# andewx/dieselfluid

Measured on AMD Instinct MI355X. Metric: M particle-steps/sec, 16M-particle WCSPH dam-break; % HBM roofline, higher is better.
Workload: dtype f32; 1 GPU; WCSPH dam-break, 16003008 particles (n3=252), h=2dx, uniform-grid neighbours, density + pressure/viscosity force + integrate + walls, math=fast; particles=16003008, parallelism=single GPU

## Files before the change

bindings/go/dslsph/dslsph.go:

```go
package dslsph

import "C"

import (
	"errors"
	"fmt"
	"unsafe"
)

var bufferIDs = map[string]C.int{
	"positions":  C.DSL_BUF_POSITIONS,
	"velocities": C.DSL_BUF_VELOCITIES,
	"forces":     C.DSL_BUF_FORCES,
	"densities":  C.DSL_BUF_DENSITIES,
	"pressures":  C.DSL_BUF_PRESSURES,
	"temps":      C.DSL_BUF_PCI_POSITIONS,
}

var auxBuffers = map[string]bool{"sizes": true, "floats": true, "sampler": true, "vecs": true}

type Engine struct {
	h      *C.dsl_handle
	Params C.dsl_params
}
// ... 323 lines not shown
	default:
		rc = C.DSL_ERR_INVALID
	}
	if rc == 0 {
		rc = C.dsl_sync(h)
	}
	if rc == 0 {
		x <- 103
	} else {
		x <- 102
	}
}

func (cp *ComputeGPU) PassIntBuffer(cpu_buffer []int, name string) error {
	if !auxBuffers[name] {
		return cp.isregistered(name)
	}
	p := &cp.eng.Params
	if name == "sizes" && len(cpu_buffer) >= 2 && (C.int32_t(cpu_buffer[0]) != p.n_particles || C.int32_t(cpu_buffer[1]) != p.n_boundary) {
		return errors.New("sizes block {N, Nboundary, ..} does not match the engine's parameters")
	}
	cp.log += "Passed Integer Buffer " + name + "\n"
	return nil
}
func (cp *ComputeGPU) ReadIntBuffer(cpu_buffer []int, name string) error {
	p := &cp.eng.Params
	switch name {
	case "sizes":
		v := [4]int{int(p.n_particles), int(p.n_boundary), int(p.lsh_buckets), int(p.lsh_bucket_size)}
		copy(cpu_buffer, v[:])
		return nil
	case "sampler":
		t := make([]int32, len(cpu_buffer))
		if len(t) == 0 {
			return nil
		}
		if err := cp.eng.ck(C.dsl_lsh_download_table(cp.eng.h, (*C.int32_t)(unsafe.Pointer(&t[0])), C.size_t(len(t)))); err != nil {
			return err
		}
		for k := range t {
			cpu_buffer[k] = int(t[k])
		}
		return nil
	}
	return fmt.Errorf("buffer [%s] holds no integers", name)
}

func (cp *ComputeGPU) RegisterGLBuffer(gl_buffer_id uint32, size int, name string) error {
	if name != "positions" {
		return errors.New("only the positions buffer has a render hand-off")
	}
	cp.registered[name] = size
	cp.log += fmt.Sprintf("RegisterGLBuffer() - buffer %s (GL id %d): read the device arrays through DevicePointers()\n", name, gl_buffer_id)
	return nil
}

func (cp *ComputeGPU) RegisterKernel(name string) bool {
	ok := name == "compute_density" || name == "predict_correct"
	if ok {
		cp.kernels[name] = true
	}
	return ok
}
func (cp *ComputeGPU) Set(d Descriptor)       { *cp.desc = d }
func (cp *ComputeGPU) Get() Descriptor        { return *cp.desc }
func (cp *ComputeGPU) HasDeviceContext() bool { return cp.eng != nil && cp.eng.h != nil }
func (cp *ComputeGPU) ValidState() bool       { return cp.HasDeviceContext() }
func (cp *ComputeGPU) Log() string            { return cp.log }


func Version() string { return C.GoString(C.dsl_version()) }

func (e *Engine) GetParams() (C.dsl_params, error) {
	var p C.dsl_params
	err := e.ck(C.dsl_get_params(e.h, &p))
	return p, err
}
const (
	OptSkin            = int(C.DSL_OPT_SKIN)
	OptSkinSteps       = int(C.DSL_OPT_SKIN_STEPS)
	OptSkinRebuilds    = int(C.DSL_OPT_SKIN_REBUILDS)
	OptSkinSuspensions = int(C.DSL_OPT_SKIN_SUSPENSIONS)
	OptSkinPredict     = int(C.DSL_OPT_SKIN_PREDICT)
	OptDeviceBytes     = int(C.DSL_OPT_DEVICE_BYTES)
	OptGridOversub     = int(C.DSL_OPT_GRID_OVERSUB)
	OptColliderTriangles = int(C.DSL_OPT_COLLIDER_TRIANGLES)
	OptCollideHits       = int(C.DSL_OPT_COLLIDE_HITS)
	OptCollideCull       = int(C.DSL_OPT_COLLIDE_CULL)
	OptCollideIndex        = int(C.DSL_OPT_COLLIDE_INDEX)
	OptCollideIndexEdge    = int(C.DSL_OPT_COLLIDE_INDEX_EDGE)
	OptCollideIndexCells   = int(C.DSL_OPT_COLLIDE_INDEX_CELLS)
	OptCollideIndexEntries = int(C.DSL_OPT_COLLIDE_INDEX_ENTRIES)
	OptCollideVisits       = int(C.DSL_OPT_COLLIDE_VISITS)
	OptCollideFullWaves    = int(C.DSL_OPT_COLLIDE_FULL_WAVES)
	OptCollideSlab = int(C.DSL_OPT_COLLIDE_SLAB)
)

func (e *Engine) SetOption(option int, value float64) error {
	return e.ck(C.dsl_set_option(e.h, C.int(option), C.double(value)))
}
func (e *Engine) GetOption(option int) (float64, error) {
	var v C.double
	err := e.ck(C.dsl_get_option(e.h, C.int(option), &v))
	return float64(v), err
}

func (e *Engine) ResetForces() error { return e.ck(C.dsl_reset_forces(e.h)) }
func (e *Engine) ForcePass() error   { return e.ck(C.dsl_force_pass(e.h)) }

func (e *Engine) SetStream(hipStream unsafe.Pointer) error { return e.ck(C.dsl_set_stream(e.h, hipStream)) }
func (e *Engine) UseOwnStream() error                      { return e.ck(C.dsl_use_own_stream(e.h)) }

func (e *Engine) Count() (live, owned int, err error) {
	var a, b C.int
	err = e.ck(C.dsl_get_count(e.h, &a, &b))
	return int(a), int(b), err
}

func (e *Engine) TimingEnable(mode int) error { return e.ck(C.dsl_timing_enable(e.h, C.int(mode))) }
func (e *Engine) TimingReset() error          { return e.ck(C.dsl_timing_reset(e.h)) }
func (e *Engine) Timing(kernelID int) (avgMs float64, launches int64, err error) {
	var ms C.double
	var n C.int64_t
	err = e.ck(C.dsl_timing_get(e.h, C.int(kernelID), &ms, &n))
	return float64(ms), int64(n), err
}

func (e *Engine) DownloadSorted(buffer C.int, out []float32) error {
	return e.ck(C.dsl_download_sorted(e.h, buffer, (*C.float)(unsafe.Pointer(&out[0])), C.size_t(len(out))))
}
func (e *Engine) DownloadIDs(out []int32) error {
	return e.ck(C.dsl_download_ids(e.h, (*C.int32_t)(unsafe.Pointer(&out[0])), C.size_t(len(out))))
}
func (e *Engine) DownloadCellStart(out []int32) error {
	return e.ck(C.dsl_download_cell_start(e.h, (*C.int32_t)(unsafe.Pointer(&out[0])), C.size_t(len(out))))
}

func SlabMessageFloats(capFull, capX int) int {
	return int(C.dsl_slab_message_floats(C.int(capFull), C.int(capX)))
}
func (e *Engine) SlabMessageFloats(capFull, capX int) int {
	return int(C.dsl_slab_message_floats_for(e.h, C.int(capFull), C.int(capX)))
}
func (e *Engine) SlabRecordFloats() int { return int(C.dsl_slab_record_floats(e.h)) }
func (e *Engine) SlabSplit(width, margin float32) error {
	return e.ck(C.dsl_slab_split(e.h, C.float(width), C.float(margin)))
}
func (e *Engine) ForcePassSplit(phase int) error { return e.ck(C.dsl_force_pass_split(e.h, C.int(phase))) }
func (e *Engine) SlabPack(widthFull, width float32, devLo, devHi unsafe.Pointer, capFull, capX int) error {
	return e.ck(C.dsl_slab_pack(e.h, C.float(widthFull), C.float(width), (*C.float)(devLo), (*C.float)(devHi), C.int(capFull), C.int(capX)))
}
func (e *Engine) SlabPackBand(widthFull float32, devLo, devHi unsafe.Pointer, capFull, capX int, stream unsafe.Pointer) error {
	return e.ck(C.dsl_slab_pack_band(e.h, C.float(widthFull), (*C.float)(devLo), (*C.float)(devHi), C.int(capFull), C.int(capX), stream))
}
func (e *Engine) SlabAppend(devMsg unsafe.Pointer, capFull, capX int) error {
	return e.ck(C.dsl_slab_append(e.h, (*C.float)(devMsg), C.int(capFull), C.int(capX)))
}
func (e *Engine) SlabAppend2(devMsgA, devMsgB unsafe.Pointer, capFull, capX int) error {
	return e.ck(C.dsl_slab_append2(e.h, (*C.float)(devMsgA), (*C.float)(devMsgB), C.int(capFull), C.int(capX)))
}

func (e *Engine) SlabStatus(resetHighWater bool) (st [4]int32, err error) {
	r := C.int(0)
	if resetHighWater {
		r = 1
	}
// ... 130 lines not shown
```

dieselfluid_amd/csrc/dslsph.hip:

```cpp
#include "../../include/dslsph.h"

#include <hip/hip_runtime.h>

#include <algorithm>
#include <climits>
#include <cmath>
#include <cstdio>
#include <cstdlib>
#include <cstring>
#include <new>
#include <string>
#include <type_traits>
#include <utility>
#include <vector>

#include "kernels_lsh.hpp"
#include "kernels_tiled.hpp"
#include "kernels_skin.hpp"
#include "engine.hpp"

using namespace dsl;

namespace {
std::string g_create_error;
// ... 538 lines not shown
    hipLaunchKernelGGL(k_update, dim3(grid_for(launch_n(h))), dim3(kBlock), 0, h->stream, c, bnd_of(h), p, v, f, uni, h->dstats,
                       xs);
  });
  if (rc) return rc;
  h->col_stage = 1;
  h->forces_uniform = true;
  h->press_zero = true;
  h->grid_valid = false;
  h->masks_valid = false;
  return DSL_OK;
}

int host_count(dsl_handle* h, int* out) {
  if (!h->c.n_ptr) {
    *out = h->n;
    return DSL_OK;
  }
  HIP_TRY(h, hipMemcpyAsync(out, h->dn, sizeof(int), hipMemcpyDeviceToHost, h->stream));
  HIP_TRY(h, hipStreamSynchronize(h->stream));
  h->n = *out;
  return DSL_OK;
}

struct BufArrays {
  int comps;
  float* a[3];
};
BufArrays buf_arrays(dsl_handle* h, int buffer) {
  auto three = [](Soa3 s) { return BufArrays{3, {s.x, s.y, s.z}}; };
  switch (buffer) {
    case DSL_BUF_POSITIONS: return three(mpos(h, h->cur_pv));
    case DSL_BUF_VELOCITIES: return three(mvel(h, h->cur_pv));
    case DSL_BUF_FORCES: return three(mfrc(h));
    case DSL_BUF_PCI_POSITIONS: return three(mpcip(h));
    case DSL_BUF_PCI_VELOCITIES: return three(mpciv(h));
    case DSL_BUF_DENSITIES: return BufArrays{1, {h->rho, nullptr, nullptr}};
    case DSL_BUF_PRESSURES: return BufArrays{1, {h->press, nullptr, nullptr}};
    default: return BufArrays{0, {nullptr, nullptr, nullptr}};
  }
}

void free_all(dsl_handle* h) {
  for (int w = 0; w < 2; ++w) {
    for (int k = 0; k < 6; ++k) {
      (void)hipFree(h->pv[w][k]);
      (void)hipFree(h->pci[w][k]);
    }
    for (int k = 0; k < 3; ++k) (void)hipFree(h->frc[w][k]);
    if (w == 0)
      for (int k = 0; k < 3; ++k) {
        (void)hipFree(h->gterm[k]);
        (void)hipFree(h->xsph[k]);
      }
    (void)hipFree(h->ids[w]);
  }
  (void)hipFree(h->rho);
  (void)hipFree(h->pterm);
  (void)hipFree(h->press);
  (void)hipFree(h->scratch1);
  (void)hipFree(h->rank);
  (void)hipFree(h->sort_keys);
  (void)hipFree(h->cell_keys_alloc);
  (void)hipFree(h->sort_work);
  (void)hipFree(h->unordered);
  (void)hipFree(h->cell_count);
  (void)hipFree(h->cell_start);
  (void)hipFree(h->block_sums);
  (void)hipFree(h->qcount);
  (void)hipFree(h->qstart);
  (void)hipFree(h->qsums);
  (void)hipFree(h->qrec);
  (void)hipFree(h->qtiles);
  (void)hipFree(h->n_qtiles);
  (void)hipFree(h->qtile_desc);
  (void)hipFree(h->qrows);
  (void)hipFree(h->qslot);
  (void)hipFree(h->pci_drift);
  if (h->pci_drift_host) (void)hipHostFree(h->pci_drift_host);
  if (h->ev_drift) (void)hipEventDestroy(h->ev_drift);
  (void)hipFree(h->skin_state);
  (void)hipFree(h->walk_ctr);
  (void)hipFree(h->lists);
  for (int k = 0; k < 6; ++k) (void)hipFree(h->pvz[k]);
  for (int k = 0; k < 3; ++k) (void)hipFree(h->pvr[k]);
  (void)hipFree(h->stage);
  (void)hipFree(h->dstats);
  (void)hipFree(h->dcounter);
  (void)hipFree(h->dn);
  (void)hipFree(h->pack_counts);
  (void)hipFree(h->tiles);
  (void)hipFree(h->tile_desc_of);
  (void)hipFree(h->tile_desc);
  (void)hipFree(h->n_tiles);
  (void)hipFree(h->hashv);
  (void)hipFree(h->bucket_of);
  (void)hipFree(h->lsh_table);
  (void)hipFree(h->lsh_len);
  (void)hipFree(h->lsh_samples);
  (void)hipFree(h->nmask);
  (void)hipFree(h->col_rec);
  (void)hipFree(h->col_box);
  (void)hipFree(h->col_chunk);
  (void)hipFree(h->col_hits);
  (void)hipFree(h->col_query);
  col_index_free(h);
  for (hipEvent_t e : h->pool) (void)hipEventDestroy(e);
  for (auto& v : h->pending)
    for (auto& pr : v) {
      (void)hipEventDestroy(pr.first);
      (void)hipEventDestroy(pr.second);
    }
  if (h->ev_band) (void)hipEventDestroy(h->ev_band);
  if (h->own_stream) (void)hipStreamDestroy(h->own_stream);
}

int alloc_pci(dsl_handle* h) {
  for (int k = 0; k < 3; ++k)
    if (!h->gterm[k])
      if (int rc = dev_alloc(h, &h->gterm[k], (size_t)h->cap)) return rc;
  for (int k = 0; k < 3; ++k)
    if (!h->xsph[k])
      if (int rc = dev_alloc(h, &h->xsph[k], (size_t)h->cap)) return rc;
  for (int w = 0; w < 2; ++w)
    for (int k = 0; k < 6; ++k)
      if (!h->pci[w][k])
        if (int rc = dev_alloc(h, &h->pci[w][k], (size_t)h->cap)) return rc;
  if (!h->pci_drift)
    if (int rc = dev_alloc(h, &h->pci_drift, (size_t)512)) return rc;
  if (!h->pci_drift_host) HIP_TRY(h, hipHostMalloc((void**)&h->pci_drift_host, 512 * sizeof(unsigned int), hipHostMallocDefault));
  if (!h->ev_drift) HIP_TRY(h, hipEventCreateWithFlags(&h->ev_drift, hipEventDisableTiming));
  return DSL_OK;
}

bool pci_tiled(const dsl_handle* h);
int alloc_query_bins(dsl_handle* h) {
  int rc = DSL_OK;
  if (!h->qcount && (rc = dev_alloc(h, &h->qcount, (size_t)h->ncell_pad))) return rc;
  if (!h->qstart && (rc = dev_alloc(h, &h->qstart, (size_t)h->ncell_pad))) return rc;
  if (!h->qsums && (rc = dev_alloc(h, &h->qsums, (size_t)h->nscan))) return rc;
  if (!h->qrec && (rc = dev_alloc(h, &h->qrec, (size_t)h->cap))) return rc;
  if (pci_tiled(h)) {
    if (!h->qtiles && (rc = dev_alloc(h, &h->qtiles, (size_t)h->tg.ntiles))) return rc;
    if (!h->n_qtiles && (rc = dev_alloc(h, &h->n_qtiles, (size_t)8))) return rc;
    if (!h->qtile_desc && (rc = dev_alloc(h, &h->qtile_desc, (size_t)std::min(h->tg.ntiles, h->cap) * kMetaInts))) return rc;
    if (h->pci_qrows && h->pci_qpair && h->pci_qtiled && !h->qrows && !side_array_fits(h, (size_t)h->ncell * kQueryRow * sizeof(float4)))
      h->pci_qrows = false;
    if (h->pci_qrows && h->pci_qpair && h->pci_qtiled && !h->qrows) {
      if (dev_alloc(h, &h->qrows, (size_t)h->ncell * kQueryRow) != DSL_OK) {
        h->qrows = nullptr;
        h->pci_qrows = false;
        h->err.clear();
        (void)hipGetLastError();
      }
    }
    if (h->qrows && h->pci_qincr && !h->qslot && (size_t)h->ncell * kQueryRow < ((size_t)1 << 31))
      if ((rc = dev_alloc(h, &h->qslot, (size_t)h->cap))) return rc;
  }
  return DSL_OK;
}

}

const char* dsl_version(void) { return "dslsph 0.1 (gfx950)"; }

const char* dsl_last_error(dsl_handle* h) { return h ? h->err.c_str() : g_create_error.c_str(); }

int dsl_params_reference(dsl_params* p, int n3) {
// ... 513 lines not shown
    if (curl)
      hipLaunchKernelGGL((k_field_div_curl<F, kOpCurl>), dim3(grid_for(n)), dim3(kBlock), 0, h->stream, h->c,
                         neigh(h), bnd_of(h), p, t, h->rho, out);
    else
      hipLaunchKernelGGL((k_field_div_curl<F, kOpDiv>), dim3(grid_for(n)), dim3(kBlock), 0, h->stream, h->c,
                         neigh(h), bnd_of(h), p, t, h->rho, out);
  });
  HIP_TRY(h, hipGetLastError());
  const int* ids = h->ids[h->cur_ids];
  if (curl) hipLaunchKernelGGL(k_pack3, dim3(grid_for(n)), dim3(kBlock), 0, h->stream, n, h->stage, ids, out.x, out.y, out.z, 0);
  else hipLaunchKernelGGL(k_pack1, dim3(grid_for(n)), dim3(kBlock), 0, h->stream, n, h->stage, ids, out.x, 0);
  HIP_TRY(h, hipGetLastError());
  HIP_TRY(h, hipMemcpyAsync(host_out, h->stage, count * sizeof(float), hipMemcpyDeviceToHost, h->stream));
  HIP_TRY(h, hipStreamSynchronize(h->stream));
  return DSL_OK;
}

int dsl_field_divergence(dsl_handle* h, int tensor_buffer, float* host_out, size_t count) {
  return field_div_curl(h, tensor_buffer, host_out, count, false);
}
int dsl_field_curl(dsl_handle* h, int tensor_buffer, float* host_out, size_t count) {
  return field_div_curl(h, tensor_buffer, host_out, count, true);
}

static int scalar_field_id(int buffer) {
  return buffer == DSL_BUF_DENSITIES ? 0 : (buffer == DSL_BUF_PRESSURES ? 1 : -1);
}

int dsl_field_laplacian(dsl_handle* h, int scalar_buffer, float* host_out, size_t count) {
  CHECK_HANDLE(h);
  int n = 0;
  if (int rc = field_prepare(h, &n)) return rc;
  const int field = scalar_field_id(scalar_buffer);
  if (!host_out || count != (size_t)n_fluid_of(h) || field < 0) return fail(h, DSL_ERR_INVALID, "dsl_field_laplacian: bad argument");
  CSoa3 p = cpos(h);
  by_math(h, [&](auto fast) {
    hipLaunchKernelGGL((k_field_laplacian<decltype(fast)::value>), dim3(grid_for(n)), dim3(kBlock), 0, h->stream, h->c,
                       neigh(h), bnd_of(h), p, h->rho, field, h->scratch1);
  });
  hipLaunchKernelGGL(k_pack1, dim3(grid_for(n)), dim3(kBlock), 0, h->stream, n, h->stage, h->ids[h->cur_ids], h->scratch1, 0);
  HIP_TRY(h, hipGetLastError());
  HIP_TRY(h, hipMemcpyAsync(host_out, h->stage, count * sizeof(float), hipMemcpyDeviceToHost, h->stream));
  HIP_TRY(h, hipStreamSynchronize(h->stream));
  return DSL_OK;
}

int dsl_field_interpolate(dsl_handle* h, int scalar_buffer, const float* host_positions, size_t npos, float* host_out) {
  CHECK_HANDLE(h);
  int n = 0;
  if (int rc = field_prepare(h, &n)) return rc;
  const int field = scalar_field_id(scalar_buffer);
  if (!host_positions || !host_out || field < 0) return fail(h, DSL_ERR_INVALID, "dsl_field_interpolate: bad argument");
  if (npos > (size_t)h->cap) return fail(h, DSL_ERR_INVALID, "dsl_field_interpolate: at most `capacity` query positions per call");
  if (npos == 0) return DSL_OK;
  CSoa3 p = cpos(h);
  HIP_TRY(h, hipMemcpyAsync(h->stage, host_positions, npos * 3 * sizeof(float), hipMemcpyHostToDevice, h->stream));
  by_math(h, [&](auto fast) {
    hipLaunchKernelGGL((k_field_interpolate<decltype(fast)::value>), dim3(grid_for((int)npos)), dim3(kBlock), 0, h->stream,
                       h->c, neigh(h), p, h->rho, field, (int)npos, h->stage, h->scratch1);
  });
  HIP_TRY(h, hipGetLastError());
  HIP_TRY(h, hipMemcpyAsync(host_out, h->scratch1, npos * sizeof(float), hipMemcpyDeviceToHost, h->stream));
  HIP_TRY(h, hipStreamSynchronize(h->stream));
  return DSL_OK;
}

namespace {
constexpr int kSkinLook = 32;
constexpr int kSkinRetry = 2048;

bool skin_usable(const dsl_handle* h) {
  return h->skin > 0.0f && h->steps >= h->skin_retry_at && h->prm.math_mode == DSL_MATH_FAST && !h->lsh && h->c.slab_axis < 0 && !h->c.n_ptr && h->nb == 0 &&
         h->col_tri == 0 &&
         !h->pci_active && h->c.xsph_eps == 0.0f && h->c.st_kappa == 0.0f && use_tiled(h) && h->nmask != nullptr &&
         (h->c.wcsph_pressure_force != 0 || h->c.wcsph_viscosity != 0);
}

int skin_alloc(dsl_handle* h) {
  int rc = DSL_OK;
  if (!h->skin_state && (rc = dev_alloc(h, &h->skin_state, 1))) return rc;
  if (!h->lists && (rc = dev_alloc(h, &h->lists, (size_t)kLMaxChunks * h->cap))) return rc;
  for (int k = 0; k < 6; ++k)
    if (!h->pvz[k] && (rc = dev_alloc(h, &h->pvz[k], (size_t)h->cap))) return rc;
  for (int k = 0; k < 3; ++k)
    if (!h->pvr[k] && (rc = dev_alloc(h, &h->pvr[k], (size_t)h->cap))) return rc;
  return DSL_OK;
}

int skin_enter(dsl_handle* h) {
  if (int rc = skin_alloc(h)) return rc;
  if (h->sort_scratch_dirty) {
    if (int rc = clean_sort_scratch(h)) return rc;
    h->sort_scratch_dirty = false;
  }
  if (int rc = set_cell_edge(h, h->c.h * (1.0f + h->skin), 3)) return rc;
  if (h->tg.ntiles > h->alloc_ntiles) {
    (void)set_cell_edge(h, h->c.h);
    return fail(h, DSL_ERR_INVALID, "skin step: the tile grid outgrew its allocation");
  }
  SkinState init{};
  init.ids_sel = h->cur_ids;
  init.force = 1;
  init.budget = 0.5f * h->skin * h->c.h * (1.0f - 1.0e-3f);
  init.dt = h->c.dt;
  init.n_live = h->n;
  init.predict = h->skin_predict;
  init.vmax2_bits = 0x7f800000u;
  HIP_TRY(h, hipMemcpyAsync(h->skin_state, &init, sizeof(init), hipMemcpyHostToDevice, h->stream));
  HIP_TRY(h, hipStreamSynchronize(h->stream));
  h->skin_live = true;
  h->skin_live_steps = 0;
  return DSL_OK;
}

int skin_step(dsl_handle* h) {
  const DevConsts& c = h->c;
  SkinState* st = h->skin_state;
  const SkinGate gate{st};
  const int n = h->n;
  const int X = h->cur_pv, Y = X ^ 1;
  const CSoa3 pX = cpos(h), vX = cvel(h);
  const CSoa3 pZ{h->pvz[0], h->pvz[1], h->pvz[2]}, vZ{h->pvz[3], h->pvz[4], h->pvz[5]};
  const CSoa3 pR{h->pvr[0], h->pvr[1], h->pvr[2]};
  const Soa3 pRw{h->pvr[0], h->pvr[1], h->pvr[2]};
  const bool ordered = sort_ordered(h);
  hipLaunchKernelGGL(k_skin_decide, dim3(1), dim3(1), 0, h->stream, st);
  HIP_TRY(h, hipGetLastError());
  int rc = timed(h, DSL_K_CELL_RANK, [&] {
    hipLaunchKernelGGL((k_cell_rank<false, true>), dim3(std::min(grid_for((n + kRankUnroll - 1) / kRankUnroll), 4096)), dim3(kBlock), 0, h->stream, c, pX.x, pX.y, pX.z,
                       ordered ? h->ids[0] : nullptr, h->rank, h->cell_count, h->unordered, nullptr, nullptr,
                       ordered ? h->cell_keys : nullptr, h->dcounter + 3, nullptr, 0, gate, h->ids[1], vX);
  });
  if (rc) return rc;
  rc = timed(h, DSL_K_SCAN, [&] { launch_scan(h, h->cell_count, h->block_sums, h->cell_start, h->dstats, h->n_tiles, gate); });
  if (rc) return rc;
  ScatterArrays a{};
  for (int k = 0; k < 6; ++k) {
    a.src[k] = h->pv[X][k];
    a.dst[k] = h->pvz[k];
  }
  a.nf = 6;
  a.ids_src = h->ids[0];
  a.ids_dst = h->ids[1];
  ScatterOrder so{ordered ? h->unordered : nullptr, h->sort_keys, reinterpret_cast<unsigned char*>(h->sort_work), nullptr,
                  ordered ? h->cell_keys : nullptr, h->dcounter + 3};
  rc = timed(h, DSL_K_SCATTER, [&] {
    hipLaunchKernelGGL(HIP_KERNEL_NAME(k_scatter<true, 6>), dim3(std::min(grid_for((n + kScatterUnroll - 1) / kScatterUnroll), 4096)), dim3(kBlock), 0, h->stream, c, a, so, pX, h->rank, h->cell_start, gate,
                       vX, pRw);
    if (ordered)
      hipLaunchKernelGGL(k_scatter_ordered<true>, dim3(h->cell_keys ? std::min(grid_for(n), 1024) : grid_for(n)), dim3(kBlock), 0,
                         h->stream, c, a, so, pX, h->rank, h->cell_start, gate, vX, pRw);
  });
  if (rc) return rc;
  rc = timed(h, DSL_K_TILE_LIST, [&] { launch_tile_tables(h, nullptr, gate); });
  if (rc) return rc;
  const double reach = 1.0 + (double)h->skin;
  const float wide_thr = (float)(1.0 - reach * reach * 1.0004 - 1.0e-4);
  rc = timed(h, DSL_K_NEIGH_LISTS, [&] {
    hipLaunchKernelGGL((k_density_pair<true, true>), dim3(persistent_grid(h, 8, true)), dim3(kPBlock), 0, h->stream, c, h->tg,
                       h->tile_desc_of, h->n_tiles, h->tile_desc, h->cell_start, bnd_of(h), pR, h->rho, h->pterm, h->nmask,
                       h->cap, wide_thr, gate);
    if (h->list_build_lockstep)
      hipLaunchKernelGGL(k_list_build, dim3(persistent_grid(h, 2, true)), dim3(kLBlock), 0, h->stream, c, h->tg, h->tile_desc_of,
                         h->n_tiles, h->tile_desc, h->nmask, h->cap, h->lists, h->cap, st, gate, pR, wide_thr);
    else
      hipLaunchKernelGGL(k_list_build_v1, dim3(persistent_grid(h, 2, true)), dim3(kLBlock), 0, h->stream, c, h->tg, h->tile_desc_of,
                         h->n_tiles, h->tile_desc, h->nmask, h->cap, h->lists, h->cap, st, gate, pR, wide_thr);
  });
  if (rc) return rc;
  rc = timed(h, DSL_K_DENSITY, [&] {
    hipLaunchKernelGGL(k_density_list, dim3(persistent_grid(h, 3, true)), dim3(kLBlock), 0, h->stream, c, h->tg, h->tile_desc_of,
                       h->n_tiles, h->tile_desc, h->cell_start, st, pX, pZ, h->lists, h->cap, h->rho, h->pterm);
  });
  if (rc) return rc;
  const Soa3 po = mpos(h, Y), vo = mvel(h, Y);
  const bool G = c.wcsph_pressure_force != 0, V = c.wcsph_viscosity != 0;
  rc = timed(h, DSL_K_FORCE_INTEGRATE, [&] {
    dim3 g(persistent_grid(h, 2, true)), b(kLBlock);
    int* wql = walk_ctr_of(h, kSiteForceList);
    with_flag(G, [&](auto fg) { with_flag(V, [&](auto fv) { with_flag(wql != nullptr, [&](auto fq) {
      constexpr bool GG = decltype(fg)::value, VV = decltype(fv)::value || !GG;
      hipLaunchKernelGGL((k_force_list<GG, VV, decltype(fq)::value>), g, b, 0, h->stream, c, h->tg, h->tile_desc_of, h->n_tiles,
                         h->tile_desc, h->cell_start, st, pX, vX, pZ, vZ, pR, h->rho, h->pterm, h->lists, h->cap, po, vo, h->dstats,
                         wql);
    }); }); });
  });
  if (rc) return rc;
  h->cur_pv = Y;
  h->masks_valid = false;
  h->grid_valid = false;
  h->dens_fresh = h->dens_held = true;
  h->forces_uniform = true;
  h->press_zero = true;
  h->skin_live_steps += 1;
  if (h->skin_live_steps % kSkinLook == 0 || h->skin_live_steps == 2) {
    int give_up = 0;
    HIP_TRY(h, hipMemcpyAsync(&give_up, &st->give_up, sizeof(int), hipMemcpyDeviceToHost, h->stream));
    HIP_TRY(h, hipStreamSynchronize(h->stream));
    if (give_up) {
      h->skin_retry_at = h->steps + 1 + ((int64_t)kSkinRetry << std::min(h->skin_suspensions, 4));
      h->skin_suspensions += 1;
      return skin_settle(h);
    }
  }
  return DSL_OK;
}

}

namespace dsl {
int skin_settle(dsl_handle* h) {
  SkinState s{};
  HIP_TRY(h, hipMemcpyAsync(&s, h->skin_state, sizeof(s), hipMemcpyDeviceToHost, h->stream));
  HIP_TRY(h, hipStreamSynchronize(h->stream));
  h->cur_ids = s.ids_sel & 1;
  h->skin_steps_total += s.n_steps;
  h->skin_rebuilds_total += s.n_rebuilds;
  h->skin_list_overflow |= s.list_overflow != 0;
  h->skin_live = false;
  h->dens_held = false;
  h->dens_fresh = false;
  return set_cell_edge(h, h->c.h);
}
}

int dsl_wcsph_step(dsl_handle* h, int nsteps) {
  CHECK_HANDLE_ONLY(h);
  for (int s = 0; s < nsteps; ++s) {
    if (skin_usable(h) && (h->skin_live || h->forces_uniform)) {
      if (!h->skin_live)
        if (int rc = skin_enter(h)) return rc;
      if (int rc = skin_step(h)) return rc;
      h->steps++;
      continue;
    }
    if (h->skin_live)
      if (int rc = skin_settle(h)) return rc;
    if (int rc = build_grid(h, false)) return rc;
    if (int rc = density_pass(h)) return rc;
    if (int rc = force_integrate(h)) return rc;
    if (int rc = collide_pass(h)) return rc;
    h->steps++;
  }
  return DSL_OK;
}

int dsl_set_option(dsl_handle* h, int option, double value) {
  CHECK_HANDLE(h);
  switch (option) {
    case DSL_OPT_SKIN:
      if (!(value >= 0.0 && value <= 0.2)) return fail(h, DSL_ERR_INVALID, "dsl_set_option: DSL_OPT_SKIN is a fraction of h in [0, 0.2]");
      h->skin = (float)value;
      h->skin_retry_at = 0;
      return DSL_OK;
    case DSL_OPT_SKIN_PREDICT:
      if (!(value >= 0.0 && value <= 0.95)) return fail(h, DSL_ERR_INVALID, "dsl_set_option: DSL_OPT_SKIN_PREDICT is a fraction of the displacement budget in [0, 0.95]");
      h->skin_predict = (float)value;
      return DSL_OK;
    case DSL_OPT_DENSITY_PAIR: h->density_pair = value != 0.0; return DSL_OK;
    case DSL_OPT_CELL_KEYS:
      h->cell_keys = value != 0.0 ? h->cell_keys_alloc : nullptr;
      h->grid_valid = false;
      return DSL_OK;
    case DSL_OPT_PERSISTENT_BLOCKS:
      if (!(value >= 0.0 && value <= 65536.0)) return fail(h, DSL_ERR_INVALID, "dsl_set_option: DSL_OPT_PERSISTENT_BLOCKS is a workgroup count (0 = no cap)");
      h->max_persistent_blocks = (int)value;
      return DSL_OK;
    case DSL_OPT_TILE_BOX: {
      const int v = (int)value, bx = v & 255, by = (v >> 8) & 255, bz = (v >> 16) & 255;
      if (value < 0.0 || value >= 16777216.0 || (v != 0 && (bx == 0 || by == 0 || bz == 0)))
        return fail(h, DSL_ERR_INVALID, "dsl_set_option: DSL_OPT_TILE_BOX is bx | by << 8 | bz << 16 (all three positive), or 0");
      h->tile_box[0] = bx;
      h->tile_box[1] = by;
      h->tile_box[2] = bz;
      h->grid_valid = false;
      h->masks_valid = false;
      return set_tile_grid(h);
    }
    case DSL_OPT_PCI_QTILED: h->pci_qtiled = value != 0.0; return DSL_OK;
    case DSL_OPT_PCI_QPAIR: h->pci_qpair = value != 0.0; return DSL_OK;
    case DSL_OPT_PCI_QROWS: h->pci_qrows = value != 0.0; return DSL_OK;
    case DSL_OPT_LIST_BUILD: h->list_build_lockstep = value != 0.0; return DSL_OK;
    case DSL_OPT_TILE_QUEUE:
      if (!(value == 0.0 || value == 1.0 || value == 2.0)) return fail(h, DSL_ERR_INVALID, "dsl_set_option: DSL_OPT_TILE_QUEUE is 0, 1 or 2");
      h->tile_queue = (int)value;
      return DSL_OK;
    case DSL_OPT_GRID_OVERSUB:
      if (!(value >= 1.0 && value <= 64.0)) return fail(h, DSL_ERR_INVALID, "dsl_set_option: DSL_OPT_GRID_OVERSUB is a factor in [1, 64]");
      h->grid_oversub = (int)value;
      return DSL_OK;
    case DSL_OPT_PCI_QINCR:
      h->pci_qincr = value != 0.0;
      h->pci_rows_live = false;
      return DSL_OK;
    case DSL_OPT_COLLIDE_CULL: h->col_cull = value != 0.0; return DSL_OK;
    case DSL_OPT_COLLIDE_SLAB:
      if (value == 0.0 && h->col_slab && h->c.n_ptr && h->col_tri > 0)
        return fail(h, DSL_ERR_INVALID, "dsl_set_option: DSL_OPT_COLLIDE_SLAB cannot go back to 0 while a slab handle holds a "
                                        "collider mesh; remove the mesh (T = 0) or leave slab mode first");
      h->col_slab = value != 0.0;
      return DSL_OK;
    case DSL_OPT_COLLIDE_INDEX: {
      const bool on = value != 0.0;
      if (on == h->col_ix_on) return DSL_OK;
      const int rc = col_index_update(h, on, h->col_ix_edge_req);
      if (rc != DSL_ERR_INVALID) h->col_ix_on = on;
      return rc;
    }
    case DSL_OPT_COLLIDE_INDEX_EDGE: {
      const float edge = (float)value;
      if (!(value >= 0.0) || !std::isfinite(edge) || (value > 0.0 && !(edge > 0.0f)))
        return fail(h, DSL_ERR_INVALID, "dsl_set_option: DSL_OPT_COLLIDE_INDEX_EDGE is a positive finite cell edge within the index's "
                                        "budget (2^22 cells, max(2^20, 64 T) list entries), or 0 for the library's choice");
      int rc = DSL_OK;
      if (h->col_ix_on && h->col_tri > 0 && edge != h->col_ix_edge_req) rc = col_index_update(h, true, edge);
      if (rc != DSL_ERR_INVALID) h->col_ix_edge_req = edge;
      return rc;
    }
    default:
      return fail(h, DSL_ERR_INVALID, "dsl_set_option: unknown or read-only option");
  }
}

int dsl_get_option(dsl_handle* h, int option, double* value) {
  CHECK_HANDLE_ONLY(h);
  if (!value) return fail(h, DSL_ERR_INVALID, "dsl_get_option: null output");
  SkinState s{};
  if (h->skin_live && (option == DSL_OPT_SKIN_STEPS || option == DSL_OPT_SKIN_REBUILDS || option == DSL_OPT_SKIN_LIST_OVERFLOW ||
                       option == DSL_OPT_SKIN_FIELDS_OWN || option == DSL_OPT_SKIN_FIELDS_PADDED || option == DSL_OPT_SKIN_TAU_STEPS)) {
    HIP_TRY(h, hipMemcpyAsync(&s, h->skin_state, sizeof(s), hipMemcpyDeviceToHost, h->stream));
    HIP_TRY(h, hipStreamSynchronize(h->stream));
  }
  switch (option) {
    case DSL_OPT_SKIN: *value = h->skin; return DSL_OK;
    case DSL_OPT_SKIN_STEPS: *value = (double)(h->skin_steps_total + s.n_steps); return DSL_OK;
    case DSL_OPT_SKIN_REBUILDS: *value = (double)(h->skin_rebuilds_total + s.n_rebuilds); return DSL_OK;
    case DSL_OPT_SKIN_LIST_OVERFLOW: *value = (h->skin_list_overflow || s.list_overflow != 0) ? 1.0 : 0.0; return DSL_OK;
    case DSL_OPT_SKIN_SUSPENSIONS: *value = (double)h->skin_suspensions; return DSL_OK;
    case DSL_OPT_DEVICE_BYTES: *value = (double)h->dev_bytes; return DSL_OK;
    case DSL_OPT_SKIN_FIELDS_OWN: *value = (double)s.fields_own; return DSL_OK;
    case DSL_OPT_SKIN_FIELDS_PADDED: *value = (double)s.fields_padded; return DSL_OK;
    case DSL_OPT_SKIN_PREDICT: *value = h->skin_predict; return DSL_OK;
    case DSL_OPT_SKIN_TAU_STEPS: *value = s.dt > 0.0f ? (double)s.tau / (double)s.dt : 0.0; return DSL_OK;
    case DSL_OPT_DENSITY_PAIR: *value = h->density_pair ? 1.0 : 0.0; return DSL_OK;
    case DSL_OPT_CELL_KEYS: *value = h->cell_keys != nullptr ? 1.0 : 0.0; return DSL_OK;
    case DSL_OPT_PERSISTENT_BLOCKS: *value = (double)h->max_persistent_blocks; return DSL_OK;
    case DSL_OPT_TILE_BOX: *value = (double)(h->tile_box[0] | (h->tile_box[1] << 8) | (h->tile_box[2] << 16)); return DSL_OK;
    case DSL_OPT_PCI_QTILED: *value = h->pci_qtiled ? 1.0 : 0.0; return DSL_OK;
    case DSL_OPT_PCI_QPAIR: *value = h->pci_qpair ? 1.0 : 0.0; return DSL_OK;
    case DSL_OPT_PCI_QROWS: *value = h->pci_qrows ? 1.0 : 0.0; return DSL_OK;
    case DSL_OPT_LIST_BUILD: *value = h->list_build_lockstep ? 1.0 : 0.0; return DSL_OK;
    case DSL_OPT_GRID_OVERSUB: *value = (double)h->grid_oversub; return DSL_OK;
    case DSL_OPT_TILE_QUEUE: *value = (double)h->tile_queue; return DSL_OK;
    case DSL_OPT_PCI_QINCR: *value = h->pci_qincr ? 1.0 : 0.0; return DSL_OK;
    case DSL_OPT_COLLIDER_TRIANGLES: *value = (double)h->col_tri; return DSL_OK;
    case DSL_OPT_COLLIDE_CULL: *value = h->col_cull ? 1.0 : 0.0; return DSL_OK;
    case DSL_OPT_COLLIDE_SLAB: *value = h->col_slab ? 1.0 : 0.0; return DSL_OK;
    case DSL_OPT_COLLIDE_HITS: {
      int hits = 0;
      if (h->col_hits) {
        HIP_TRY(h, hipMemcpyAsync(&hits, h->col_hits, sizeof(int), hipMemcpyDeviceToHost, h->stream));
        HIP_TRY(h, hipStreamSynchronize(h->stream));
      }
      *value = (double)hits;
      return DSL_OK;
    }
    case DSL_OPT_COLLIDE_INDEX: *value = h->col_ix_on ? 1.0 : 0.0; return DSL_OK;
    case DSL_OPT_COLLIDE_INDEX_EDGE: *value = h->col_ix_cells > 0 ? (double)h->col_ix.edge : 0.0; return DSL_OK;
    case DSL_OPT_COLLIDE_INDEX_CELLS: *value = (double)h->col_ix_cells; return DSL_OK;
    case DSL_OPT_COLLIDE_INDEX_ENTRIES: *value = (double)h->col_ix_entries; return DSL_OK;
    case DSL_OPT_COLLIDE_VISITS:
    case DSL_OPT_COLLIDE_FULL_WAVES: {
      unsigned long long ctr[2] = {0, 0};
      if (!h->col_last_indexed || h->col_ix_cells == 0) {
        *value = -1.0;
        return DSL_OK;
      }
      HIP_TRY(h, hipMemcpyAsync(ctr, h->col_ix.counters, sizeof(ctr), hipMemcpyDeviceToHost, h->stream));
      HIP_TRY(h, hipStreamSynchronize(h->stream));
      *value = (double)ctr[option == DSL_OPT_COLLIDE_VISITS ? 0 : 1];
      return DSL_OK;
    }
    default: return fail(h, DSL_ERR_INVALID, "dsl_get_option: unknown option");
  }
}

int dsl_pcisph_begin(dsl_handle* h) {
  CHECK_HANDLE(h);
  if (int rc = alloc_pci(h)) return rc;
  const size_t n = (size_t)h->cap;
  for (int k = 0; k < 6; ++k)
    HIP_TRY(h, hipMemcpyAsync(h->pci[h->cur_pci][k], h->pv[h->cur_pv][k], n * sizeof(float), hipMemcpyDeviceToDevice,
                              h->stream));
  h->pci_active = true;
  if (h->pci_steps != 0) HIP_TRY(h, hipMemsetAsync(h->pci_drift, 0, 512 * sizeof(unsigned int), h->stream));
  h->pci_steps = 0;
  h->pci_binned = false;
  if (h->drift_pending) HIP_TRY(h, hipEventSynchronize(h->ev_drift));
  h->drift_pending = false;
  HIP_TRY(h, hipMemsetAsync(&h->dstats->pci_escaped, 0, sizeof(int), h->stream));
  return DSL_OK;
}

namespace {
constexpr int kPciDriftPeriod = 4;
constexpr double kPciDriftFraction = 0.002;

int pci_drift_check(dsl_handle* h) {
  if (h->pci_bin_mode != 0 || h->pci_binned || h->lsh || h->pci_steps == 0 || h->pci_steps % kPciDriftPeriod != 0) return DSL_OK;
  hipStreamCaptureStatus capturing = hipStreamCaptureStatusNone;
  if (hipStreamIsCapturing(h->stream, &capturing) == hipSuccess && capturing != hipStreamCaptureStatusNone) return DSL_OK;
  if (h->drift_pending) {
    HIP_TRY(h, hipEventSynchronize(h->ev_drift));
    h->drift_pending = false;
    unsigned long long left = 0, all = 0;
    for (int k = 0; k < 256; ++k) {
      left += h->pci_drift_host[k];
      all += h->pci_drift_host[256 + k];
    }
    if (all != 0 && (double)left > kPciDriftFraction * (double)all) {
      h->pci_binned = true;
      return DSL_OK;
    }
  }
  HIP_TRY(h, hipMemcpyAsync(h->pci_drift_host, h->pci_drift, 512 * sizeof(unsigned int), hipMemcpyDeviceToHost, h->stream));
// ... 544 lines not shown
```

dieselfluid_amd/csrc/engine.hpp:

```cpp
#pragma once

#include "../../include/dslsph.h"

#include <hip/hip_runtime.h>

#include <string>
#include <utility>
#include <vector>

#include "collide.hpp"

struct SlabLink;

namespace dsl {
constexpr float kSkinPredict = 0.8f;
}

struct dsl_handle {
  int device = 0;
  hipStream_t own_stream = nullptr, stream = nullptr;
  dsl_params prm{};
  dsl::DevConsts c{};
  int n = 0, cap = 0, ncell = 0, ncell_pad = 0, nscan = 0;
  int nb = 0;
  float b0_pos[3] = {0.f, 0.f, 0.f};
  bool ids_global = false;
  int* dcounter = nullptr;
  int* dn = nullptr;
  int* pack_counts = nullptr;
  float split_margin = 0.0f, split_width = 0.0f;
  bool split_pending = false;
  bool pci_split_guard = false;
  hipEvent_t ev_band = nullptr;
  bool lsh = false;
  int lsh_bits = 0, lsh_cap = 0;
  float* hashv = nullptr;
  int *bucket_of = nullptr, *lsh_table = nullptr, *lsh_len = nullptr, *lsh_samples = nullptr;
  dsl::TileGrid tg{};
  int *tiles = nullptr, *n_tiles = nullptr;
  int *tile_desc_of = nullptr, *tile_desc = nullptr;
  float* pv[2][6] = {};
  int* ids[2] = {};
  float* frc[2][3] = {};
  float* pci[2][6] = {};
  float *rho = nullptr, *pterm = nullptr, *press = nullptr, *scratch1 = nullptr;
  float* gterm[3] = {};
  int pci_bin_mode = 0;
  int build_seq = 0;
  bool qcount_dirty = false;
  bool pci_counters_clean = false;
  bool pci_iter_pending = false;
  bool pci_binned = false;
  bool pci_qpair = true;
  bool pci_qtiled = true;
  int64_t pci_steps = 0;
  int *qcount = nullptr, *qstart = nullptr, *qsums = nullptr;
  int *qtiles = nullptr, *n_qtiles = nullptr, *qtile_desc = nullptr;
  float4* qrows = nullptr;
  bool pci_qrows = true;
  int* qslot = nullptr;
  bool pci_qincr = true;
  bool pci_rows_live = false;
  float4* qrec = nullptr;
  unsigned int* pci_drift = nullptr;
  unsigned int* pci_drift_host = nullptr;
  hipEvent_t ev_drift = nullptr;
  bool drift_pending = false;
  float* xsph[3] = {};
  unsigned int* nmask = nullptr;
  bool masks_valid = false;
  int *rank = nullptr, *cell_count = nullptr, *cell_start = nullptr, *block_sums = nullptr;
  unsigned int* unordered = nullptr;
  int *sort_keys = nullptr, *sort_work = nullptr;
  int* cell_keys = nullptr;
  int* cell_keys_alloc = nullptr;
  float* stage = nullptr;
  dsl::DevStats* dstats = nullptr;
  int cur_pv = 0, cur_ids = 0, cur_f = 0, cur_pci = 0;
  bool grid_valid = false, forces_uniform = false, press_zero = true, pci_active = false, dens_fresh = false;
  bool dens_held = false;
  bool sort_scratch_dirty = false;
  bool density_pair = true;
  int max_persistent_blocks = 0;
  int64_t steps = 0;
  size_t dev_bytes = 0;
  float skin = 0.0f;
  bool skin_live = false;
  int64_t skin_steps_total = 0, skin_rebuilds_total = 0;
  bool skin_list_overflow = false;
  int64_t skin_retry_at = 0, skin_live_steps = 0;
  int skin_suspensions = 0;
  int tile_box[3] = {8, 4, 4};
  int alloc_ntiles = 0;
  int tile_tbz = dsl::kTB;
  dsl::SkinState* skin_state = nullptr;
  uint4* lists = nullptr;
  float* pvz[6] = {};
  float* pvr[3] = {};
  float skin_predict = dsl::kSkinPredict;
  bool list_build_lockstep = true;
  int grid_oversub = 8;
  int tile_queue = 1;
  int* walk_ctr = nullptr;
  int walk_parity[16] = {};
  int col_tri = 0, col_alloc = 0;
  float col_radius = 0.0f, col_rest = 0.0f, col_s_thr = -1.0f;
  bool col_cull = true;
  dsl::TriRec* col_rec = nullptr;
  dsl::TriBox *col_box = nullptr, *col_chunk = nullptr;
  int* col_hits = nullptr;
  float* col_query = nullptr;
  bool col_ix_on = false;
  float col_ix_edge_req = 0.0f;
  dsl::ColIndex col_ix{};
  int col_ix_cells = 0;
  long long col_ix_entries = 0;
  size_t col_ix_bytes = 0;
  bool col_last_indexed = false;
  bool col_slab = false;
  int col_stage = 0;
  bool col_step_zeroed = false;
  std::string err;
  SlabLink* link = nullptr;
  int timing = 0;
  std::vector<hipEvent_t> pool;
  std::vector<std::pair<hipEvent_t, hipEvent_t>> pending[DSL_K_COUNT];
  double total_ms[DSL_K_COUNT] = {};
  int64_t launches[DSL_K_COUNT] = {};
};

namespace dsl {

int fail(dsl_handle* h, int code, const std::string& msg);

#define HIP_TRY(h, expr)                                                                             \
  do {                                                                                               \
    hipError_t e__ = (expr);                                                                         \
    if (e__ != hipSuccess)                                                                           \
      return fail((h), DSL_ERR_DEVICE, std::string(#expr) + ": " + hipGetErrorString(e__));          \
  } while (0)

#define CHECK_HANDLE_ONLY(h)                              \
  do {                                                    \
    if (!(h)) return fail(nullptr, DSL_ERR_INVALID, "null handle"); \
    hipError_t e__ = hipSetDevice((h)->device);           \
    if (e__ != hipSuccess) return fail((h), DSL_ERR_DEVICE, std::string("hipSetDevice: ") + hipGetErrorString(e__)); \
  } while (0)
int skin_settle(dsl_handle* h);
#define CHECK_HANDLE(h)                                   \
  do {                                                    \
    CHECK_HANDLE_ONLY(h);                                 \
    if ((h)->skin_live)                                   \
      if (int rc__ = skin_settle(h)) return rc__;         \
  } while (0)

inline int launch_n(const dsl_handle* h) { return h->c.n_ptr ? h->cap : h->n; }

template <class T>
int dev_alloc(dsl_handle* h, T** p, size_t count) {
  hipError_t e = hipMalloc((void**)p, count * sizeof(T) + 64);
  if (e != hipSuccess) return fail(h, DSL_ERR_NOMEM, std::string("hipMalloc: ") + hipGetErrorString(e));
  e = hipMemsetAsync(*p, 0, count * sizeof(T) + 64, h->stream);
  if (e != hipSuccess) return fail(h, DSL_ERR_DEVICE, std::string("hipMemsetAsync: ") + hipGetErrorString(e));
  h->dev_bytes += count * sizeof(T) + 64;
  return DSL_OK;
}

hipEvent_t get_event(dsl_handle* h);

template <class F>
int timed(dsl_handle* h, int kid, F&& launch) {
  if (h->timing == 1 || (h->timing == 2 && (kid == DSL_K_DENSITY || kid == DSL_K_FORCE_INTEGRATE || kid == DSL_K_PCI_DENSITY))) {
    hipEvent_t a = get_event(h), b = get_event(h);
    (void)hipEventRecord(a, h->stream);
    launch();
    (void)hipEventRecord(b, h->stream);
    h->pending[kid].emplace_back(a, b);
  } else {
    launch();
  }
  hipError_t e = hipGetLastError();
  if (e != hipSuccess) return fail(h, DSL_ERR_DEVICE, std::string("kernel launch: ") + hipGetErrorString(e));
// ... 41 lines not shown
```

dieselfluid_amd/csrc/kernels_grid.hpp:

```cpp
#pragma once

#include <climits>

#include "sph_device.hpp"

namespace dsl {

constexpr int kBlock = 256;
constexpr int kCellKeys = 32;
#ifndef DSL_RANK_UNROLL
#define DSL_RANK_UNROLL 2
#endif
constexpr int kRankUnroll = DSL_RANK_UNROLL;
constexpr int kScanTile = 4096;

__device__ __forceinline__ int sort_cell(const DevConsts& c, float x, float y, float z) {
  if (c.slab_axis >= 0 && !((x == x) && (y == y) && (z == z))) return c.ncell;
  return cell_of(c, x, y, z);
}

__device__ __forceinline__ float skin_ref(float x, float v, float tau) { return __builtin_fmaf(tau, v, x); }

template <bool OFF_GRID, bool REF = false>
__global__ __launch_bounds__(kBlock) void k_cell_rank(DevConsts c, const float* __restrict__ px,
// ... 123 lines not shown
  for (int k = 0; k < 4; ++k) {
    const int4 v = src[k * kBlock + threadIdx.x];
    s += (v.x + v.y) + (v.z + v.w);
  }
  int total;
  block_exclusive_scan(s, lds, total);
  if (threadIdx.x == 0) block_sums[blockIdx.x] = total;
}

__global__ __launch_bounds__(kBlock) void k_scan_apply(int* __restrict__ count,
                                                       const int* __restrict__ block_sums,
                                                       int* __restrict__ cell_start, DevStats* stats,
                                                       SkinGate gate = SkinGate{nullptr}) {
  __shared__ int carry_sums[kBlock / kWave];
  __shared__ int wave_sums[4][kBlock / kWave];
  if (gate.closed()) return;
  const int lane = threadIdx.x & (kWave - 1), wid = threadIdx.x >> 6;
  int4* src = reinterpret_cast<int4*>(count + (size_t)blockIdx.x * kScanTile);
  int4* dst = reinterpret_cast<int4*>(cell_start + (size_t)blockIdx.x * kScanTile);
  int4 v[4];
#pragma unroll
  for (int k = 0; k < 4; ++k) v[k] = src[k * kBlock + threadIdx.x];
  int part = 0;
  for (int i = threadIdx.x; i < (int)blockIdx.x; i += kBlock) part += block_sums[i];
  for (int off = kWave / 2; off > 0; off >>= 1) part += __shfl_xor(part, off, kWave);
  if (lane == 0) carry_sums[wid] = part;
  int mx = 0, s4[4], inc[4];
#pragma unroll
  for (int k = 0; k < 4; ++k) {
    if ((v[k].x | v[k].y | v[k].z | v[k].w) != 0) src[k * kBlock + threadIdx.x] = make_int4(0, 0, 0, 0);
    mx = max(max(mx, max(v[k].x, v[k].y)), max(v[k].z, v[k].w));
    s4[k] = (v[k].x + v[k].y) + (v[k].z + v[k].w);
    inc[k] = wave_inclusive_scan(s4[k]);
    if (lane == kWave - 1) wave_sums[k][wid] = inc[k];
  }
  __syncthreads();
  int carry = 0;
#pragma unroll
  for (int w = 0; w < kBlock / kWave; ++w) carry += carry_sums[w];
#pragma unroll
  for (int k = 0; k < 4; ++k) {
    int off = 0, tot = 0;
#pragma unroll
    for (int w = 0; w < kBlock / kWave; ++w) {
      const int t = wave_sums[k][w];
      if (w < wid) off += t;
      tot += t;
    }
    const int ex = carry + off + inc[k] - s4[k];
    int4 o;
    o.x = ex;
    o.y = ex + v[k].x;
    o.z = o.y + v[k].y;
    o.w = o.z + v[k].z;
    dst[k * kBlock + threadIdx.x] = o;
    carry += tot;
  }
  for (int off = kWave / 2; off > 0; off >>= 1) mx = max(mx, __shfl_xor(mx, off, kWave));
  if (stats != nullptr && (threadIdx.x & (kWave - 1)) == 0 && mx > 0 &&
      mx > __hip_atomic_load(&stats->max_cell_count, __ATOMIC_RELAXED, __HIP_MEMORY_SCOPE_AGENT))
    atomicMax(&stats->max_cell_count, mx);
}

constexpr int kMaxScatter = 16;
struct ScatterArrays {
  const float* src[kMaxScatter];
  float* dst[kMaxScatter];
  int nf;
  const int* ids_src;
  int* ids_dst;
};

struct ScatterOrder {
  const unsigned int* unordered;
  int* keys;
  unsigned char* later;
  int* dest;
  const int* cell_keys;
  const int* overfull;
};

struct SortPos {
  float x, y, z;
};
template <bool REF>
__device__ __forceinline__ SortPos sort_pos(const CSoa3& pos, const CSoa3& vel, float tau, int i) {
  if constexpr (REF) return SortPos{skin_ref(pos.x[i], vel.x[i], tau), skin_ref(pos.y[i], vel.y[i], tau), skin_ref(pos.z[i], vel.z[i], tau)};
  return SortPos{pos.x[i], pos.y[i], pos.z[i]};
}
template <bool REF>
__device__ __forceinline__ void scatter_move(const ScatterArrays& a, const ScatterOrder& o, int i, int d, int id,
                                             int* __restrict__ ids_dst, const Soa3& ref, const SortPos& sp) {
  ids_dst[d] = id;
  for (int f = 0; f < a.nf; ++f) a.dst[f][d] = a.src[f][i];
  if constexpr (REF) {
    ref.x[d] = sp.x;
    ref.y[d] = sp.y;
    ref.z[d] = sp.z;
  }
  if (o.dest) o.dest[i] = d;
}

struct ScatterIds {
  const int* src;
  int* dst;
};
__device__ __forceinline__ ScatterIds skin_ids(const ScatterArrays& a, const SkinGate& gate) {
  const bool swap_ids = gate.st != nullptr && gate.st->ids_sel == 0;
  return ScatterIds{swap_ids ? a.ids_dst : a.ids_src, swap_ids ? const_cast<int*>(a.ids_src) : a.ids_dst};
}
template <int NFMAX>
struct ScatterPayload {
  float v[NFMAX];
};
template <int NFMAX>
__device__ __forceinline__ void scatter_fetch(const ScatterArrays& a, int i, ScatterPayload<NFMAX>& p) {
#pragma unroll
  for (int f = 0; f < NFMAX; ++f) {
    p.v[f] = 0.0f;
    if (NFMAX == 6 || f < a.nf) p.v[f] = a.src[f][i];
  }
}
template <bool REF, int NFMAX>
__device__ __forceinline__ void scatter_store(const ScatterArrays& a, const ScatterOrder& o, int i, int d, int id,
                                              int* __restrict__ ids_dst, const Soa3& ref, const SortPos& sp,
                                              const ScatterPayload<NFMAX>& p) {
  ids_dst[d] = id;
#pragma unroll
  for (int f = 0; f < NFMAX; ++f)
    if (NFMAX == 6 || f < a.nf) a.dst[f][d] = p.v[f];
  if constexpr (REF) {
    ref.x[d] = sp.x;
    ref.y[d] = sp.y;
    ref.z[d] = sp.z;
  }
  if (o.dest) o.dest[i] = d;
}

#ifndef DSL_SCATTER_UNROLL
#define DSL_SCATTER_UNROLL 2
#endif
constexpr int kScatterUnroll = DSL_SCATTER_UNROLL;
template <bool REF = false, int NFMAX = kMaxScatter>
__global__ __launch_bounds__(kBlock) void k_scatter(DevConsts c, ScatterArrays a, ScatterOrder o, CSoa3 pos,
                                                    const int* __restrict__ rank,
                                                    const int* __restrict__ cell_start, SkinGate gate = SkinGate{nullptr},
                                                    CSoa3 vel = CSoa3{nullptr, nullptr, nullptr},
                                                    Soa3 ref = Soa3{nullptr, nullptr, nullptr}) {
  constexpr int U = kScatterUnroll;
  if (gate.closed()) return;
  const ScatterIds ids = skin_ids(a, gate);
  const int* ids_src = ids.src;
  int* ids_dst = ids.dst;
  const float tau = REF ? gate.st->tau : 0.0f;
  const int n = live_n(c);
  const bool pos_in_payload = a.nf >= (REF ? 6 : 3) && pos.x == a.src[0] && pos.y == a.src[1] && pos.z == a.src[2] &&
                              (!REF || (vel.x == a.src[3] && vel.y == a.src[4] && vel.z == a.src[5]));
  for (int first = blockIdx.x * (U * kBlock) + threadIdx.x; first < n; first += gridDim.x * (U * kBlock)) {
  ScatterPayload<NFMAX> pay[U];
  int id[U], r[U], cell[U], s[U], e[U], d[U];
  unsigned int uword[U];
  SortPos sp[U];
  bool in[U], later[U];
#pragma unroll
  for (int u = 0; u < U; ++u) {
    in[u] = first + u * kBlock < n;
    const int i = min(first + u * kBlock, n - 1);
    scatter_fetch<NFMAX>(a, i, pay[u]);
    id[u] = ids_src[i];
    r[u] = rank[i];
    if (pos_in_payload) {
      if constexpr (REF) sp[u] = SortPos{skin_ref(pay[u].v[0], pay[u].v[3], tau), skin_ref(pay[u].v[1], pay[u].v[4], tau), skin_ref(pay[u].v[2], pay[u].v[5], tau)};
      else sp[u] = SortPos{pay[u].v[0], pay[u].v[1], pay[u].v[2]};
    } else {
      sp[u] = sort_pos<REF>(pos, vel, tau, i);
    }
  }
#pragma unroll
  for (int u = 0; u < U; ++u) {
    cell[u] = sort_cell(c, sp[u].x, sp[u].y, sp[u].z);
    const int cc = min(cell[u], c.ncell - 1);
    s[u] = cell_start[cc];
    e[u] = cell_start[cc + 1];
    uword[u] = o.unordered != nullptr ? o.unordered[cc >> 5] : 0u;
  }
#pragma unroll
  for (int u = 0; u < U; ++u) {
    d[u] = s[u] + r[u];
    later[u] = in[u] && cell[u] != c.ncell && ((uword[u] >> (cell[u] & 31)) & 1u) != 0u;
    if (later[u] && o.cell_keys != nullptr) {
      const int cnt = e[u] - s[u];
      if (cnt <= kCellKeys) {
        const int4* row = reinterpret_cast<const int4*>(o.cell_keys + (size_t)cell[u] * kCellKeys);
        int below = 0;
        for (int k0 = 0; k0 < cnt; k0 += 8) {
          const int4 v = row[k0 / 4], w = row[k0 / 4 + 1];
          const int key[8] = {v.x, v.y, v.z, v.w, w.x, w.y, w.z, w.w};
#pragma unroll
          for (int q = 0; q < 8; ++q)
            below += (k0 + q < cnt && (key[q] < id[u] || (key[q] == id[u] && k0 + q < r[u]))) ? 1 : 0;
        }
        d[u] = s[u] + below;
        later[u] = false;
      }
    }
  }
#pragma unroll
  for (int u = 0; u < U; ++u) {
    const int i = first + u * kBlock;
    if (!in[u]) continue;
    if (cell[u] != c.ncell) {
      if (later[u]) o.keys[d[u]] = id[u];
      else scatter_store<REF, NFMAX>(a, o, i, d[u], id[u], ids_dst, ref, sp[u], pay[u]);
    }
    if (o.unordered != nullptr && o.cell_keys == nullptr) o.later[i] = later[u] ? 1 : 0;
  }
  }
}

template <bool REF = false>
__global__ __launch_bounds__(kBlock) void k_scatter_ordered(DevConsts c, ScatterArrays a, ScatterOrder o, CSoa3 pos,
                                                            const int* __restrict__ rank,
                                                            const int* __restrict__ cell_start,
                                                            SkinGate gate = SkinGate{nullptr},
                                                            CSoa3 vel = CSoa3{nullptr, nullptr, nullptr},
                                                            Soa3 ref = Soa3{nullptr, nullptr, nullptr}) {
  if (gate.closed()) return;
  const ScatterIds ids = skin_ids(a, gate);
  const float tau = REF ? gate.st->tau : 0.0f;
  if (o.cell_keys != nullptr) {
    if (*o.overfull == 0) return;
    const int n = live_n(c);
    for (int i = blockIdx.x * kBlock + threadIdx.x; i < n; i += gridDim.x * kBlock) {
      const SortPos sp = sort_pos<REF>(pos, vel, tau, i);
      const int cell = sort_cell(c, sp.x, sp.y, sp.z);
      if (cell == c.ncell) continue;
      const int s = cell_start[cell], e = cell_start[cell + 1];
      if (e - s <= kCellKeys || !((o.unordered[cell >> 5] >> (cell & 31)) & 1u)) continue;
      const int id = ids.src[i], mine = s + rank[i];
      int below = 0;
      for (int k = s; k < e; ++k) {
        const int key = o.keys[k];
        below += (key < id || (key == id && k < mine)) ? 1 : 0;
      }
      scatter_move<REF>(a, o, i, s + below, id, ids.dst, ref, sp);
    }
    return;
  }
  const int i = blockIdx.x * kBlock + threadIdx.x;
  if (i >= live_n(c) || !o.later[i]) return;
  const SortPos sp = sort_pos<REF>(pos, vel, tau, i);
  const int cell = sort_cell(c, sp.x, sp.y, sp.z);
  const int id = ids.src[i];
  const int s = cell_start[cell], e = cell_start[cell + 1], mine = s + rank[i];
  int below = 0;
  for (int k0 = s; k0 < e; k0 += 8) {
    int key[8];
#pragma unroll
    for (int u = 0; u < 8; ++u) key[u] = k0 + u < e ? o.keys[k0 + u] : INT_MAX;
#pragma unroll
    for (int u = 0; u < 8; ++u) below += (key[u] < id || (key[u] == id && k0 + u < mine)) ? 1 : 0;
  }
  scatter_move<REF>(a, o, i, s + below, id, ids.dst, ref, sp);
}

__global__ __launch_bounds__(kBlock) void k_permute1(DevConsts c, const int* __restrict__ dest, CSoa3 pos,
                                                     const float* __restrict__ src, float* __restrict__ dst) {
  const int i = blockIdx.x * kBlock + threadIdx.x;
  if (i >= live_n(c)) return;
  if (sort_cell(c, pos.x[i], pos.y[i], pos.z[i]) == c.ncell) return;
  dst[dest[i]] = src[i];
}

__global__ __launch_bounds__(kBlock) void k_unpack3(int n, const float* __restrict__ stage, const int* __restrict__ ids,
                                                    float* __restrict__ x, float* __restrict__ y,
                                                    float* __restrict__ z, int limit, int zero_id) {
  const int s = blockIdx.x * kBlock + threadIdx.x;
  if (s >= n) return;
  const int o = ids[s];
  if (o >= limit) return;
  const bool zero = o == zero_id;
  x[s] = zero ? 0.0f : stage[3 * o];
  y[s] = zero ? 0.0f : stage[3 * o + 1];
  z[s] = zero ? 0.0f : stage[3 * o + 2];
}
__global__ __launch_bounds__(kBlock) void k_unpack1(int n, const float* __restrict__ stage, const int* __restrict__ ids,
                                                    float* __restrict__ x, int limit) {
  const int s = blockIdx.x * kBlock + threadIdx.x;
  if (s >= n) return;
  const int o = ids[s];
  if (o < limit) x[s] = stage[o];
}
__global__ __launch_bounds__(kBlock) void k_append_boundary(int nb, int at, int first_id, int zero_id,
                                                            const float* __restrict__ stage, float* __restrict__ x,
                                                            float* __restrict__ y, float* __restrict__ z,
                                                            float* __restrict__ vx, float* __restrict__ vy,
                                                            float* __restrict__ vz, int* __restrict__ ids, Soa3 pcip,
                                                            Soa3 pciv, float* __restrict__ rho,
                                                            float* __restrict__ pterm) {
  const int k = blockIdx.x * kBlock + threadIdx.x;
  if (k >= nb) return;
  const int d = at + k;
  rho[d] = 0.0f;
  pterm[d] = __uint_as_float(0x7fc00000u);
  const bool zero = first_id + k == zero_id;
  const float px = zero ? 0.0f : stage[3 * k], py = zero ? 0.0f : stage[3 * k + 1], pz = zero ? 0.0f : stage[3 * k + 2];
  x[d] = px;
  y[d] = py;
  z[d] = pz;
  vx[d] = 0.0f;
  vy[d] = 0.0f;
  vz[d] = 0.0f;
  ids[d] = first_id + k;
  if (pcip.x != nullptr) {
    pcip.x[d] = px;
    pcip.y[d] = py;
    pcip.z[d] = pz;
    pciv.x[d] = 0.0f;
    pciv.y[d] = 0.0f;
    pciv.z[d] = 0.0f;
  }
}
__global__ __launch_bounds__(kBlock) void k_pack3(int n, float* __restrict__ stage, const int* __restrict__ ids,
                                                  const float* __restrict__ x, const float* __restrict__ y,
                                                  const float* __restrict__ z, int sorted_order) {
  const int s = blockIdx.x * kBlock + threadIdx.x;
  if (s >= n) return;
  const int o = sorted_order ? s : ids[s];
  stage[3 * o] = x[s];
  stage[3 * o + 1] = y[s];
  stage[3 * o + 2] = z[s];
}
__global__ __launch_bounds__(kBlock) void k_pack1(int n, float* __restrict__ stage, const int* __restrict__ ids,
                                                  const float* __restrict__ x, int sorted_order) {
// ... 322 lines not shown
```

dieselfluid_amd/csrc/kernels_skin.hpp:

```cpp
#pragma once

#include "kernels_tiled.hpp"

namespace dsl {

constexpr int kLEntries = 8;
constexpr int kLMaxChunks = 12;
constexpr int kLMaxEntries = kLMaxChunks * kLEntries - 1;
constexpr int kLBlock = 512;
constexpr unsigned int kLGlobal = 0xffffu;
constexpr float kSkinTauSteps = 16.0f;
constexpr int kLQuads = 14;
static_assert(kTRows * kLQuads <= kLBlock, "one quad per lane");

__global__ void k_skin_decide(SkinState* st) {
  const float d = __builtin_sqrtf(__uint_as_float(st->disp2_bits)) * (1.0f + 1.0e-6f);
  const bool rb = st->force != 0 || !(d <= st->budget);
  st->rebuild = rb ? 1 : 0;
  if (st->unlisted * 64 > st->n_live) st->give_up = 1;
  if (rb) {
    st->ids_sel ^= 1;
    st->n_rebuilds += 1;
    st->unlisted = 0;
    st->fields_own = st->fields_padded = 0u;
    const float vmax = __builtin_sqrtf(__uint_as_float(st->vmax2_bits)) * (1.0f + 1.0e-6f);
    float tau = 0.0f;
    if (st->predict > 0.0f && vmax > 0.0f && vmax < 3.0e38f) tau = fminf(st->predict * st->budget / vmax, kSkinTauSteps * st->dt);
    st->tau = tau;
  }
  st->disp = d;
  st->force = 0;
  st->disp2_bits = 0u;
  st->vmax2_bits = 0u;
  st->n_steps += 1;
  st->history = (st->history << 1) | (rb ? 1u : 0u);
  if (st->n_steps >= 16 && __builtin_popcount(st->history & 0xffffu) >= 5) st->give_up = 1;
}

__device__ __forceinline__ unsigned int pad_entry(const TileMeta& m) { return (unsigned int)(m.row_lds[1] - kTPad) << 4; }

__global__ __launch_bounds__(kLBlock) void k_list_build_v1(DevConsts c, TileGrid tg, const int* __restrict__ desc_of,
                                                        const int* __restrict__ n_tiles, const int* __restrict__ desc,
                                                        const unsigned int* __restrict__ nmask, int mstride,
                                                        uint4* __restrict__ lists, int lstride, SkinState* st,
                                                        SkinGate gate, CSoa3 p, float wide_thr) {
  if (gate.closed()) return;
  __shared__ TileMeta metas[2];
  constexpr int kLStaged = 8;
  __shared__ uint4 held[kLStaged][kLBlock];
  __shared__ unsigned int tile_fields[2];
  const int tid = threadIdx.x;
  if (tid < 2) tile_fields[tid] = 0u;
  TileFeed feed(desc_of, *n_tiles);
  int di = 0;
  bool have = feed.pop(di);
  if (have) tile_meta_store(metas[0], tile_meta_request(desc, di));
  for (int cur = 0; have; cur ^= 1) {
    const TileMeta& m = metas[cur];
    sync_lds();
    have = feed.pop(di);
    int table_word = 0;
    if (have) table_word = tile_meta_request(desc, di);
    const int ntarg = m.tprefix[kTB * kTB];
    const unsigned int pad = pad_entry(m);
    if (m.overflow != 0 && tid == 0) atomicAdd(&st->unlisted, ntarg);
    for_each_target<true, kLBlock>(ntarg, tid, tid, [&](auto shared_c, int t, int sub, int k) {
      constexpr bool SHARED = decltype(shared_c)::value;
      if (SHARED && sub != 0) return;
      const TileTarget tt = tile_target(m, t);
      const int g = tt.g;
      unsigned int b0 = 0u, b1 = 0u, b2 = 0u, b3 = 0u;
      int n = 0;
      auto push = [&](unsigned int entry) {
        b0 = __builtin_amdgcn_alignbit(b1, b0, 16);
        b1 = __builtin_amdgcn_alignbit(b2, b1, 16);
        b2 = __builtin_amdgcn_alignbit(b3, b2, 16);
        b3 = (b3 >> 16) | (entry << 16);
        n += 1;
        if ((n & (kLEntries - 1)) == 0) {
          const int ch = (n >> 3) - 1;
          if (ch < kLStaged) held[ch][tid] = make_uint4(b0, b1, b2, b3);
          else if (ch < kLMaxChunks) lists[(size_t)ch * lstride + g] = make_uint4(b0, b1, b2, b3);
        }
      };
      auto emit = [&](int rec) {
        if (rec != tt.own) push((unsigned int)rec << 4);
      };
      const bool masks = m.overflow == 0;
      if (masks) {
        int rj[9], rje[9];
        unsigned int w1[9], w2[9];
#pragma unroll
        for (int ri = 0; ri < 9; ++ri) {
          tile_run(m, tt.srow + (ri / 3 - 1) * kTH + (ri % 3 - 1), tt.lx, rj[ri], rje[ri]);
          const int len = rje[ri] - rj[ri];
          w1[ri] = (len > 0 && len <= 64) ? nmask[(size_t)ri * mstride + g] : 0u;
          w2[ri] = (len > 32 && len <= 64) ? nmask[(size_t)(kMaskHigh + ri) * mstride + g] : 0u;
        }
        push(0u);
#pragma unroll
        for (int ri = 0; ri < 9; ++ri) {
          const int j = rj[ri], je = rje[ri], len = je - j;
          if (len > 64) {
            const int rr = tt.srow + (ri / 3 - 1) * kTH + (ri % 3 - 1);
            const int g0 = m.row_gs[rr] - m.row_lds[rr];
            const float xi = p.x[g], yi = p.y[g], zi = p.z[g];
            for (int r = j; r < je; ++r) {
              const float dx = xi - p.x[g0 + r], dy = yi - p.y[g0 + r], dz = zi - p.z[g0 + r];
              const float tq = __builtin_fmaf(-dist2<true>(dx, dy, dz), c.inv_hh, 1.0f);
              if (tq > wide_thr) emit(r);
            }
            continue;
          }
          unsigned int w = w1[ri];
          int top = j + ((min(len, 32) + 3) & ~3) - 1;
          while (w != 0u) {
            const int b = __builtin_ctz(w);
            w &= w - 1u;
            emit(top - b);
          }
          w = w2[ri];
          top = j + 32 + ((len - 32 + 3) & ~3) - 1;
          while (w != 0u) {
            const int b = __builtin_ctz(w);
            w &= w - 1u;
            emit(top - b);
          }
        }
      }
      const bool fits = masks && n <= kLMaxChunks * kLEntries;
      if (masks && !fits) st->list_overflow = 1;
      int fields = fits ? n : 0;
      const int own_fields = fields;
      if constexpr (!SHARED) {
        int wmax = 0;
#pragma unroll
        for (int bit = 6; bit >= 0; --bit) {
          const int cand = wmax | (1 << bit);
          if (__builtin_amdgcn_ballot_w64(fields >= cand) != 0ull) wmax = cand;
        }
        fields = wmax;
      }
      atomicAdd(&tile_fields[0], (unsigned int)own_fields);
      atomicAdd(&tile_fields[1], (unsigned int)(fits ? fields : 0));
      const int nch = (fields + kLEntries - 1) / kLEntries;
      if (fits)
        while (n < nch * kLEntries) push(pad);
      for (int ch = 0; ch < min(nch, kLStaged); ++ch) {
        uint4 v = held[ch][tid];
        if (ch == 0) v.x = (v.x & 0xffff0000u) | (unsigned int)fields;
        if (fits) lists[(size_t)ch * lstride + g] = v;
      }
      if (!fits) lists[g] = make_uint4(kLGlobal, 0u, 0u, 0u);
    });
    if (have) tile_meta_store(metas[cur ^ 1], table_word);
    sync_lds();
    if (tid == 0) {
      atomicAdd(&st->fields_own, tile_fields[0]);
      atomicAdd(&st->fields_padded, tile_fields[1]);
      tile_fields[0] = tile_fields[1] = 0u;
    }
  }
}

constexpr int kLQueue = 24;
__global__ __launch_bounds__(kLBlock, 4) void k_list_build(DevConsts c, TileGrid tg, const int* __restrict__ desc_of,
                                                        const int* __restrict__ n_tiles, const int* __restrict__ desc,
                                                        const unsigned int* __restrict__ nmask, int mstride,
                                                        uint4* __restrict__ lists, int lstride, SkinState* st,
                                                        SkinGate gate, CSoa3 p, float wide_thr) {
  if (gate.closed()) return;
  __shared__ TileMeta metas[2];
  __shared__ unsigned int qword[kLQueue][kLBlock];
  __shared__ unsigned short qtop[kLQueue][kLBlock];
  __shared__ unsigned int tile_fields[2];
  const int tid = threadIdx.x;
  if (tid < 2) tile_fields[tid] = 0u;
  TileFeed feed(desc_of, *n_tiles);
  int di = 0;
  bool have = feed.pop(di);
  if (have) tile_meta_store(metas[0], tile_meta_request(desc, di));
  for (int cur = 0; have; cur ^= 1) {
    const TileMeta& m = metas[cur];
    sync_lds();
    have = feed.pop(di);
    int table_word = 0;
    if (have) table_word = tile_meta_request(desc, di);
    const int ntarg = m.tprefix[kTB * kTB];
    const unsigned int pad = pad_entry(m);
    if (m.overflow != 0 && tid == 0) atomicAdd(&st->unlisted, ntarg);
    for_each_target<true, kLBlock>(ntarg, tid, tid, [&](auto shared_c, int t, int sub, int k) {
      constexpr bool SHARED = decltype(shared_c)::value;
      if (SHARED && sub != 0) return;
      const TileTarget tt = tile_target(m, t);
      const int g = tt.g;
      const bool masks = m.overflow == 0;
      int nq = 0, total = 0;
      bool too_many = false;
      auto enqueue = [&](unsigned int w, int top) {
        if (w != 0u) {
          if (nq < kLQueue) {
            qword[nq][tid] = w;
            qtop[nq][tid] = (unsigned short)top;
          } else {
            too_many = true;
          }
          nq += 1;
          total += __builtin_popcount(w);
        }
      };
      if (masks) {
        unsigned int run[9], w1[9], w2[9];
        unsigned int unmasked = 0u;
#pragma unroll
        for (int ri = 0; ri < 9; ++ri) {
          run[ri] = (unsigned int)m.run[(tt.srow + (ri / 3 - 1) * kTH + (ri % 3 - 1)) * kTB + tt.lx - 1];
          const int len = (int)(run[ri] >> 16) - (int)(run[ri] & 0xffffu);
          w1[ri] = (len > 0 && len <= 64) ? nmask[(size_t)ri * mstride + g] : 0u;
          w2[ri] = (len > 32 && len <= 64) ? nmask[(size_t)(kMaskHigh + ri) * mstride + g] : 0u;
          if (len > 64) unmasked |= 1u << ri;
        }
#pragma unroll
        for (int ri = 0; ri < 9; ++ri) {
          const int j = (int)(run[ri] & 0xffffu), len = (int)(run[ri] >> 16) - j;
          unsigned int a = w1[ri], b = w2[ri];
          const int top1 = j + ((min(len, 32) + 3) & ~3) - 1;
          const int top2 = j + 32 + ((len - 32 + 3) & ~3) - 1;
          if (ri == 4) {
            const int b1 = top1 - tt.own, b2 = top2 - tt.own;
            if (b1 >= 0 && b1 < 32) a &= ~(1u << b1);
            if (b2 >= 0 && b2 < 32) b &= ~(1u << b2);
          }
          enqueue(a, top1);
          enqueue(b, top2);
        }
        while (unmasked != 0u) {
          const int ri = __builtin_ctz(unmasked);
          unmasked &= unmasked - 1u;
          const int rr = tt.srow + (ri / 3 - 1) * kTH + (ri % 3 - 1);
          int j, je;
          tile_run(m, rr, tt.lx, j, je);
          const int g0 = m.row_gs[rr] - m.row_lds[rr];
          const float xi = p.x[g], yi = p.y[g], zi = p.z[g];
          for (int r0 = j; r0 < je; r0 += 32) {
            unsigned int w = 0u;
            const int top = r0 + 31;
            for (int r = r0; r < min(r0 + 32, je); ++r) {
              const float dx = xi - p.x[g0 + r], dy = yi - p.y[g0 + r], dz = zi - p.z[g0 + r];
              const float tq = __builtin_fmaf(-dist2<true>(dx, dy, dz), c.inv_hh, 1.0f);
              if (tq > wide_thr && r != tt.own) w |= 1u << (top - r);
            }
            enqueue(w, top);
          }
        }
      }
      const int n_own = 1 + total;
      const bool fits = masks && !too_many && n_own <= kLMaxChunks * kLEntries;
      if (masks && !fits) st->list_overflow = 1;
      int fields = fits ? n_own : 0;
      const int own_fields = fields;
      int wmax = 0;
#pragma unroll
      for (int bit = 6; bit >= 0; --bit) {
        const int cand = wmax | (1 << bit);
        if (__builtin_amdgcn_ballot_w64(fields >= cand) != 0ull) wmax = cand;
      }
      if constexpr (!SHARED) fields = fits ? wmax : 0;
      atomicAdd(&tile_fields[0], (unsigned int)own_fields);
      atomicAdd(&tile_fields[1], (unsigned int)fields);
      const int nch = (fields + kLEntries - 1) / kLEntries;
      const int nch_wave = (wmax + kLEntries - 1) / kLEntries;
      unsigned int b0 = 0u, b1 = 0u, b2 = 0u, b3 = 0u;
      unsigned int k0 = 0u, k1 = 0u, k2 = 0u, k3 = 0u;
      int qi = 0;
      unsigned int w = 0u, top = 0u;
      unsigned int wn = (fits && nq > 0) ? qword[0][tid] : 0u, tn = (fits && nq > 0) ? qtop[0][tid] : 0u;
      const int nq_live = fits ? nq : 0;
      for (int it = 0; it < nch_wave * kLEntries; ++it) {
        unsigned int entry = pad;
        if (it == 0) {
          entry = 0u;
        } else {
          if (w == 0u && qi < nq_live) {
            w = wn;
            top = tn;
            qi += 1;
            if (qi < nq_live) {
              wn = qword[qi][tid];
              tn = qtop[qi][tid];
            }
          }
          if (w != 0u) {
            const int b = __builtin_ctz(w);
            w &= w - 1u;
            entry = (top - (unsigned int)b) << 4;
          }
        }
        b0 = __builtin_amdgcn_alignbit(b1, b0, 16);
        b1 = __builtin_amdgcn_alignbit(b2, b1, 16);
        b2 = __builtin_amdgcn_alignbit(b3, b2, 16);
        b3 = (b3 >> 16) | (entry << 16);
        if ((it & (kLEntries - 1)) == kLEntries - 1) {
          const int ch = it >> 3;
          if (ch == 0) {
            k0 = b0, k1 = b1, k2 = b2, k3 = b3;
          } else if (ch < nch) {
            lists[(size_t)ch * lstride + g] = make_uint4(b0, b1, b2, b3);
          }
        }
      }
      if (fits) lists[g] = make_uint4((k0 & 0xffff0000u) | (unsigned int)fields, k1, k2, k3);
      else lists[g] = make_uint4(kLGlobal, 0u, 0u, 0u);
    });
    if (have) tile_meta_store(metas[cur ^ 1], table_word);
    sync_lds();
    if (tid == 0) {
      atomicAdd(&st->fields_own, tile_fields[0]);
      atomicAdd(&st->fields_padded, tile_fields[1]);
      tile_fields[0] = tile_fields[1] = 0u;
    }
  }
}

template <int NF, class Load4, class Store>
__device__ __forceinline__ void stage_tile(const TileMeta& m, Load4&& load4, Store&& store) {
  const int t = threadIdx.x, r = t / kLQuads, k = t - r * kLQuads;
  if (r >= kTRows) return;
  const int len = m.row_len[r], gs = m.row_gs[r], ls = m.row_lds[r];
  for (int q = k; 4 * q < len; q += kLQuads) {
    float4 v[NF];
    load4(gs + 4 * q, v);
#pragma unroll
    for (int i = 0; i < 4; ++i) {
// ... 106 lines not shown
      }
      const int g = tt.g;
      float acc = 0.0f;
      if (staged && fields != kLGlobal) {
        const float4 me = A[tt.own];
        const float two_hh = 2.0f * c.inv_hh;
        const float sx = two_hh * me.x, sy = two_hh * me.y, sz = two_hh * me.z, a0 = 1.0f + me.w;
        float acc0 = 0.0f, acc1 = 0.0f;
        float4 cq[4];
        auto fetch4 = [&](unsigned int w0, unsigned int w1) {
          cq[0] = lds_at(A, w0 & 0xffffu);
          cq[1] = lds_at(A, w0 >> 16);
          cq[2] = lds_at(A, w1 & 0xffffu);
          cq[3] = lds_at(A, w1 >> 16);
        };
        auto sum4 = [&](const float4 (&r)[4]) {
#pragma unroll
          for (int u = 0; u < 4; ++u) {
            const float q = fma_clamp01(r[u].z, sz, __builtin_fmaf(r[u].y, sy, __builtin_fmaf(r[u].x, sx, r[u].w + a0)));
            if (u & 1) acc1 = __builtin_fmaf(q, q, acc1);
            else acc0 = __builtin_fmaf(q, q, acc0);
          }
        };
        if constexpr (SHARED) {
          walk_shared(lists, lstride, g, pad, sub, k, fields, [&](const Chunk& e) {
            fetch4(e.x, e.y);
            float4 c1[4] = {cq[0], cq[1], cq[2], cq[3]};
            fetch4(e.z, e.w);
            sum4(c1);
            sum4(cq);
          });
        } else {
          const int nf = __builtin_amdgcn_readfirstlane((int)fields), nch = (nf + kLEntries - 1) >> 3;
          const uint4* lp = lists + (size_t)2 * lstride + g;
          Chunk e = q0, e1 = q1;
          fetch4(e.x, e.y);
          for (int ch = 0;;) {
            float4 c1[4] = {cq[0], cq[1], cq[2], cq[3]};
            fetch4(e.z, e.w);
            sum4(c1);
            if (8 * ch + 4 >= nf) break;
            const Chunk en = e1;
            if (ch + 2 < nch) e1 = load_chunk(lp, 0);
            lp += lstride;
            float4 c2[4] = {cq[0], cq[1], cq[2], cq[3]};
            fetch4(en.x, en.y);
            sum4(c2);
            e = en;
            ch += 1;
            if (8 * ch >= nf) break;
          }
        }
        acc = acc0 + acc1;
      } else if (sub == 0) {
        const float xi = p.x[g], yi = p.y[g], zi = p.z[g];
        float a = 0.0f;
        for_each_grid_candidate(c, cell_start, xi, yi, zi, [&](int j) {
          if (j == g) return;
          const float dx = xi - p.x[j], dy = yi - p.y[j], dz = zi - p.z[j];
          const float r2 = dist2<true>(dx, dy, dz);
          if (r2 < c.hh) {
            const float q = __builtin_fmaf(-r2, c.inv_hh, 1.0f);
            a = __builtin_fmaf(q, q, a);
          }
        });
        acc = a;
      }
      if constexpr (SHARED) {
        for (int o = 1; o < k; o <<= 1) acc += __shfl_xor(acc, o, kWave);
        if (sub != 0) return;
      }
      acc *= c.mass * c.A;
      rho[g] = acc;
      const float pr = tait_eos<true>(c, acc, c.eos_d0_grad);
      pterm[g] = acc > 0.0f ? dsl_div<true>(pr, acc * acc) : 0.0f;
    });
  }
}

template <bool WANT_G, bool WANT_V, bool QUEUE>
__global__ __launch_bounds__(kLBlock, 4) void k_force_list(DevConsts c, TileGrid tg, const int* __restrict__ desc_of,
                                                           const int* __restrict__ n_tiles, const int* __restrict__ desc,
                                                           const int* __restrict__ cell_start, SkinState* st, CSoa3 pX,
                                                           CSoa3 vX, CSoa3 pZ, CSoa3 vZ, CSoa3 pR, const float* __restrict__ rho,
                                                           const float* __restrict__ pterm,
                                                           const uint4* __restrict__ lists, int lstride, Soa3 pout,
                                                           Soa3 vout, DevStats* stats, int* __restrict__ walk_ctr) {
  __shared__ TileMeta metas[2];
  __shared__ float4 A[kTCap];
  __shared__ float4 B[kTCap];
  __shared__ int feed_slot[2];
  const int tid = threadIdx.x;
  const bool rb = st->rebuild != 0;
  const CSoa3 pin = rb ? pZ : pX, vin = rb ? vZ : vX;
  unsigned int vbits = 0u, fbits = 0u, dbits = 0u;
  typename TileSource<QUEUE>::type feed = TileSource<QUEUE>::make(desc_of, *n_tiles, walk_ctr, feed_slot);
  int di = 0;
  bool have = feed.pop(di);
  if (have) tile_meta_store(metas[0], tile_meta_request(desc, di));
  for (int cur = 0; have; cur ^= 1) {
    const TileMeta& m = metas[cur];
    sync_lds();
    have = feed.pop(di);
    int table_word = 0;
    if (have) table_word = tile_meta_request(desc, di);
    const int ntarg = m.tprefix[kTB * kTB];
    const bool staged = m.overflow == 0;
    const unsigned int pad = pad_entry(m);
    Chunk q0 = pad_chunk(pad), q1 = q0;
    const bool first_full = ntarg > kLBlock / 2;
    TileTarget tt0{0, 0, 0, 0};
    const int tperm = (tid & ~(kWave - 1)) + b128_group_slot(tid & (kWave - 1));
    if (first_full && tperm < ntarg) {
      tt0 = tile_target(m, tperm);
      q0 = load_chunk(lists, tt0.g);
      q1 = load_chunk(lists, (size_t)lstride + tt0.g);
    }
    if (staged)
      stage_tile<8>(
          m,
          [&](int gg, float4* o) {
            o[0] = load4u(pin.x + gg);
            o[1] = load4u(pin.y + gg);
            o[2] = load4u(pin.z + gg);
            o[3] = WANT_G ? load4u(pterm + gg) : make_float4(0.f, 0.f, 0.f, 0.f);
            if constexpr (WANT_V) {
              o[4] = load4u(vin.x + gg);
              o[5] = load4u(vin.y + gg);
              o[6] = load4u(vin.z + gg);
              o[7] = load4u(rho + gg);
            } else {
              o[4] = o[5] = o[6] = o[7] = make_float4(0.f, 0.f, 0.f, 0.f);
            }
          },
          [&](int slot, const float* o, bool real) {
            float4 a = make_float4(kFar, kFar, kFar, 0.f), b = make_float4(0.f, 0.f, 0.f, 0.f);
            if (real && o[0] == o[0] && o[1] == o[1] && o[2] == o[2]) {
              a = make_float4(o[0], o[1], o[2], o[3]);
              if constexpr (WANT_V) b = make_float4(o[4], o[5], o[6], o[7] > 0.0f ? __builtin_amdgcn_rcpf(o[7]) : 0.0f);
            }
            A[slot] = a;
            if constexpr (WANT_V) B[slot] = b;
          });
    if (have) tile_meta_store(metas[cur ^ 1], table_word);
    sync_lds();
    for_each_target<true, kLBlock>(ntarg, tid, tperm, [&](auto shared_c, int t, int sub, int k) {
      constexpr bool SHARED = decltype(shared_c)::value;
      TileTarget tt;
      unsigned int fields;
      if constexpr (SHARED) {
        tt = tile_target(m, t);
        fields = shared_fields(lists, tt.g, sub);
      } else {
        if (t == tperm) tt = tt0;
        else {
          tt = tile_target(m, t);
          q0 = load_chunk(lists, tt.g);
          q1 = load_chunk(lists, (size_t)lstride + tt.g);
        }
        fields = take_count(q0, pad);
      }
      const int g = tt.g;
      float px, py, pz, vx, vy, vz;
      float gx = 0.f, gy = 0.f, gz = 0.f, lx_ = 0.f, ly_ = 0.f, lz_ = 0.f, lw_ = 0.f;
      const bool listed = staged && fields != kLGlobal;
      if (listed) {
        const float4 a = A[tt.own];
        px = a.x, py = a.y, pz = a.z;
        const float pti = WANT_G ? a.w : 0.f;
        if (px == kFar) px = py = pz = __uint_as_float(0x7fc00000u);
        if constexpr (WANT_V) {
          const float4 b = B[tt.own];
          vx = b.x, vy = b.y, vz = b.z;
        } else {
          vx = vin.x[g], vy = vin.y[g], vz = vin.z[g];
        }
        if constexpr (WANT_G || WANT_V) {
          const float ninvh = -c.inv_h;
// ... 43 lines not shown
            const uint4* lp = lists + (size_t)2 * lstride + g;
            Chunk e = q0, e1 = q1;
            Pair1 p0 = fetch1(e.x & 0xffffu), p1 = fetch1(e.x >> 16);
            auto word = [&](unsigned int next_word) {
              Pair1 cu = p0;
              p0 = fetch1(next_word & 0xffffu);
              accum(cu.a, cu.b);
              cu = p1;
              p1 = fetch1(next_word >> 16);
              accum(cu.a, cu.b);
            };
            for (int ch = 0;;) {
              word(e.y);
              if (8 * ch + 2 >= nf) break;
              word(e.z);
              if (8 * ch + 4 >= nf) break;
              word(e.w);
              if (8 * ch + 6 >= nf) break;
              const Chunk en = e1;
              if (ch + 2 < nch) e1 = load_chunk(lp, 0);
              lp += lstride;
              word(en.x);
              e = en;
              ch += 1;
              if (8 * ch >= nf) break;
            }
          }
        }
      } else {
        px = pin.x[g], py = pin.y[g], pz = pin.z[g];
        vx = vin.x[g], vy = vin.y[g], vz = vin.z[g];
        if (sub == 0) {
          float accG[3] = {0.f, 0.f, 0.f}, accV[3] = {0.f, 0.f, 0.f};
          if constexpr (WANT_G || WANT_V)
            force_sweep<true, WANT_G, WANT_V>(c, grid_neigh(cell_start), g, pin, vin, rho, pterm, accG, accV, nullptr, nullptr);
          gx = accG[0], gy = accG[1], gz = accG[2];
          lx_ = accV[0], ly_ = accV[1], lz_ = accV[2];
        }
      }
      if constexpr (SHARED) {
        for (int o = 1; o < k; o <<= 1) {
          gx += __shfl_xor(gx, o, kWave);
          gy += __shfl_xor(gy, o, kWave);
          gz += __shfl_xor(gz, o, kWave);
          lx_ += __shfl_xor(lx_, o, kWave);
          ly_ += __shfl_xor(ly_, o, kWave);
          lz_ += __shfl_xor(lz_, o, kWave);
          lw_ += __shfl_xor(lw_, o, kWave);
        }
        if (sub != 0) return;
      }
      if (listed) {
        if constexpr (WANT_V) {
          lx_ = __builtin_fmaf(-vx, lw_, lx_);
          ly_ = __builtin_fmaf(-vy, lw_, ly_);
          lz_ = __builtin_fmaf(-vz, lw_, lz_);
        }
        const float sg = -c.B;
        gx *= sg;
        gy *= sg;
        gz *= sg;
        const float sv = c.C * c.mass;
        lx_ *= sv;
        ly_ *= sv;
        lz_ *= sv;
      }
      float fx = c.reset[0], fy = c.reset[1], fz = c.reset[2];
      if constexpr (WANT_G) {
        const float dm = rho[g] * c.mass * c.pressure_sign;
        fx = __builtin_fmaf(gx, dm, fx);
        fy = __builtin_fmaf(gy, dm, fy);
        fz = __builtin_fmaf(gz, dm, fz);
      }
      if constexpr (WANT_V) {
        fx = __builtin_fmaf(lx_, c.mu, fx);
        fy = __builtin_fmaf(ly_, c.mu, fy);
        fz = __builtin_fmaf(lz_, c.mu, fz);
      }
      fx += c.ext[0];
      fy += c.ext[1];
      fz += c.ext[2];
      integrate_core(c, fx, fy, fz, px, py, pz, vx, vy, vz, vbits, fbits);
      {
        const float ex = px - pR.x[g], ey = py - pR.y[g], ez = pz - pR.z[g];
        const unsigned int db = nonneg_bits(__builtin_fmaf(ez, ez, __builtin_fmaf(ey, ey, ex * ex)));
        dbits = db > dbits ? db : dbits;
      }
      pout.x[g] = px;
      pout.y[g] = py;
      pout.z[g] = pz;
      vout.x[g] = vx;
      vout.y[g] = vy;
      vout.z[g] = vz;
    });
  }
  feed.finish();
  wave_atomic_max(&stats->max_vel_bits, vbits);
  wave_atomic_max(&stats->max_f_bits, fbits);
  wave_atomic_max(&st->disp2_bits, dbits);
  wave_atomic_max(&st->vmax2_bits, vbits);
}

}
```

dieselfluid_amd/csrc/kernels_tiled.hpp:

```cpp
#pragma once

#include "kernels_sph.hpp"

namespace dsl {

constexpr int kTH = kTB + 2;
constexpr int kTRows = kTH * kTH;
constexpr int kTBlock = 512;
constexpr int kTPad = 4;
constexpr int kTCap = 2304;
constexpr float kFar = 1.0e15f;
constexpr int kTileLists = 5;
constexpr int kMaskWords = 19;
constexpr int kMaskValid = 9, kMaskHigh = 10;

struct TileMeta {
  int4 trow[kTB * kTB];
  int row_gs[kTRows];
  int row_len[kTRows];
  int row_lds[kTRows + 1];
  int run[kTRows * kTB];
  int tprefix[kTB * kTB + 1];
  int overflow;
  int tile;
// ... 666 lines not shown
  for_each_run<false>(qrow, 0, 1, [&](int, int rr) {
    int j, je;
    tile_run(m, rr, lx, j, je);
    for (; j + 4 < je; j += 8) {
      test4(j);
      test4(j + 4);
    }
    if (j < je) test4(j);
  });
  return acc + acc1;
}
__device__ __forceinline__ float densityf_global(const DevConsts& c, const int* cell_start, const CSoa3& p, float qx,
                                                 float qy, float qz) {
  float density = c.W0;
  for_each_grid_candidate(c, cell_start, qx, qy, qz, [&](int j) {
    const float dx = qx - p.x[j], dy = qy - p.y[j], dz = qz - p.z[j];
    const float r2 = dist2<true>(dx, dy, dz);
    if (r2 < c.hh) {
      const float q = __builtin_fmaf(-r2, c.inv_hh, 1.0f);
      density = __builtin_fmaf(c.mass * c.A, q * q, density);
    }
  });
  return density;
}
__device__ __forceinline__ void pci_accumulate(const DevConsts& c, float* press, int g, float density, unsigned int& ebits) {
  const float density_error = density - c.ref_density;
  const float abs_err = density_error * __builtin_amdgcn_rcpf(c.ref_density);
  press[g] += density_error * c.delta;
  const unsigned int eb = nonneg_bits(abs_err);
  ebits = eb > ebits ? eb : ebits;
}

template <bool STAMPS, class Commit, class Sweep>
__device__ __forceinline__ void sweep_tiles_double_buffered(TileFeed& feed, const int* desc, TileMeta* metas,
                                                            float4 (*Abuf)[kTCap], const LoadPos4& load4, Commit&& commit,
                                                            Sweep&& sweep) {
  int di = 0;
  bool have = feed.pop(di);
  if (!have) return;
  tile_meta_store(metas[0], tile_meta_request(desc, di));
  bool have_next = feed.pop(di);
  int table_word = have_next ? tile_meta_request(desc, di) : 0;
  sync_lds();
  {
    StageRegs<3> sr;
    if (!metas[0].overflow) {
      stage_issue<3>(metas[0], load4, sr);
      commit(metas[0], sr, Abuf[0]);
    }
  }
  if (have_next) tile_meta_store(metas[1], table_word);
  int mc = 0, mn = 1, mnn = 2;
  for (int cur = 0; have; cur ^= 1) {
    DSL_STAMP_IF(STAMPS, d0);
    sync_lds();
    DSL_STAMP_IF(STAMPS, d1);
    DSL_STAMP_ADD_IF(STAMPS, 4, d0, d1);
    StageRegs<3> sr;
    bool have_nn = false, stage_next = false;
    table_word = 0;
    if (have_next) {
      stage_next = metas[mn].overflow == 0;
      if (stage_next) stage_issue<3>(metas[mn], load4, sr);
      have_nn = feed.pop(di);
      if (have_nn) table_word = tile_meta_request(desc, di);
    }
    DSL_STAMP_IF(STAMPS, d1b);
    DSL_STAMP_ADD_IF(STAMPS, 12, d1, d1b);
    sweep(metas[mc], Abuf[cur]);
    DSL_STAMP_IF(STAMPS, d4);
    if (stage_next) commit(metas[mn], sr, Abuf[cur ^ 1]);
    if (have_nn) tile_meta_store(metas[mnn], table_word);
    DSL_STAMP_IF(STAMPS, d5);
    DSL_STAMP_ADD_IF(STAMPS, 13, d4, d5);
    have = have_next;
    have_next = have_nn;
    const int t = mc;
    mc = mn;
    mn = mnn;
    mnn = t;
  }
}

template <int BLOCK, class Body>
__device__ __forceinline__ void sweep_tiles_pair(const DevConsts& c, TileFeed& feed, const int* desc, TileMeta* metas,
                                                 float4* A, const CSoa3& p, Body&& body) {
  const int tid = threadIdx.x;
  const LoadPos4 load4{p};
  const LoadPos1 load1{p};
  auto meta_request = [&](int desc_index, int (&w)[2]) {
#pragma unroll
    for (int k = 0; k < 2; ++k) {
      const int i = tid + k * BLOCK;
      w[k] = i < kMetaInts ? desc[(size_t)desc_index * kMetaInts + i] : 0;
    }
  };
  auto meta_store = [&](TileMeta& m, const int (&w)[2]) {
#pragma unroll
    for (int k = 0; k < 2; ++k) {
      const int i = tid + k * BLOCK;
      if (i < kMetaInts) reinterpret_cast<int*>(&m)[i] = w[k];
    }
  };
  int di = 0;
  bool have = feed.pop(di);
  if (!have) return;
  {
    int w[2];
    meta_request(di, w);
    meta_store(metas[0], w);
  }
  for (int cur = 0; have; cur ^= 1) {
    TileMeta& m = metas[cur];
    sync_lds();
    have = feed.pop(di);
    int tw[2] = {0, 0};
    if (have) meta_request(di, tw);
    const bool ovf = m.overflow != 0;
    if (!ovf) {
      const StoreTileRecord store(A, m, c.inv_hh);
      StageRegs<3> sr0, sr1;
      stage_issue<3>(m, load4, sr0, tid);
      stage_issue<3>(m, load4, sr1, tid + BLOCK);
      stage_commit<3>(m, sr0, load1, store, tid);
      stage_commit<3>(m, sr1, load1, store, tid + BLOCK);
    }
    if (have) meta_store(metas[cur ^ 1], tw);
    sync_lds();
    body(m, ovf);
  }
}
struct MaskQueue {
  unsigned int mm, n1, n2;
  int top, tp1, tp2;
  __device__ __forceinline__ void shift() {
    mm = n1;
    top = tp1;
    n1 = n2;
    tp1 = tp2;
    n2 = 0u;
  }
  __device__ __forceinline__ int take(int own, int pad_rec, bool& counts) {
    const bool has = mm != 0u;
    const int b = 31 - __builtin_clz(mm | 1u);
    const int idx = has ? top - b : pad_rec;
    mm = has ? (mm & ~(1u << b)) : 0u;
    counts = has && idx != own;
    if (mm == 0u) shift();
    return idx;
  }
};

template <bool SHARE, bool EXACT = false>
__global__ __launch_bounds__(kTBlock, 4) void k_density_tiled(DevConsts c, TileGrid tg, const int* __restrict__ desc_of,
                                                          const int* __restrict__ n_tiles, const int* __restrict__ desc,
                                                          const int* __restrict__ cell_start, Bnd bnd, CSoa3 p,
                                                          float* __restrict__ rho, float* __restrict__ pterm,
                                                          unsigned int* __restrict__ nmask, int mstride) {
#ifdef DSL_DENSITY_SINGLE_BUFFER
  constexpr bool DB = false;
#else
  constexpr bool DB = !EXACT;
#endif
  __shared__ TileMeta metas[DB ? 3 : 2];
  __shared__ float4 Abuf[DB ? 2 : 1][kTCap];
  __shared__ float4 R[EXACT ? kTCap : 1];
  const int tid = threadIdx.x, lane = tid & (kWave - 1);
  static_assert(!(EXACT && SHARE), "the exact sum is sequential: one lane per target");
  if (!EXACT && c.slab_axis < 0 && share_wanted(n_tiles) != SHARE) return;
  const LoadPos4 load4{p};
  const LoadPos1 load1{p};
  auto commit = [&](const TileMeta& mt, const StageRegs<3>& sr, float4* img) {
    const float ox = __int_as_float(mt.centre[0]), oy = __int_as_float(mt.centre[1]), oz = __int_as_float(mt.centre[2]);
    stage_commit<3>(mt, sr, load1, [&](int slot, const float* o, bool real) {
      const float4 v = tile_record(o, real, ox, oy, oz, c.inv_hh);
      if constexpr (EXACT) {
        img[slot] = real ? make_float4(o[0], o[1], o[2], 0.0f) : make_float4(kFar, kFar, kFar, 0.0f);
        R[slot] = v;
      } else {
        img[slot] = v;
      }
    });
  };
  auto sweep = [&](const TileMeta& m, const float4* __restrict__ A, bool force_global) {
    DSL_STAMP(d2);
    const bool ovf = m.overflow != 0 || force_global;
    const int ntarg = m.tprefix[kTB * kTB];
    const int tperm = (tid & ~(kWave - 1)) + b128_group_slot(lane);
    for_each_target<SHARE>(ntarg, tid, tperm, [&](auto shared_c, int t, int sub, int k) {
      constexpr bool SHARED = decltype(shared_c)::value;
      const TileTarget tt = tile_target(m, t);
      const int srow = tt.srow, g = tt.g, lx = tt.lx;
      float acc = 0.0f, acc1 = 0.0f, self_term = 1.0f;
      if constexpr (EXACT) {
        if (!ovf) {
          const int own = tt.own;
          const float4 me = A[own];
          const int pad_rec = m.row_lds[1] - kTPad;
          float density = 0.0f;
          const float4 mer = R[own];
          const float two_hh = 2.0f * c.inv_hh;
          const float qsx = two_hh * mer.x, qsy = two_hh * mer.y, qsz = two_hh * mer.z, qa0 = 1.0f + mer.w;
          const float reach = 4.0f * c.h;
          const bool far_lane = !(fabsf(mer.x) <= reach && fabsf(mer.y) <= reach && fabsf(mer.z) <= reach);
          const bool prefilter = __builtin_amdgcn_ballot_w64(far_lane) == 0ull;
          const ExactDivisor Dhh = exact_divisor_uniform(c.hh);
          auto add = [&](const float4& cnd, bool counts) {
            const float dx = me.x - cnd.x, dy = me.y - cnd.y, dz = me.z - cnd.z;
            const float dist = dsl_sqrt<false>(dist2<false>(dx, dy, dz));
            float w = 0.0f;
            if (!(dist >= c.h)) {
              const float xx = dist * dist;
              const float q = 1.0f - exact_div(xx, Dhh);
              const float aq = c.A * q;
// ... 170 lines not shown
    DSL_STAMP_ADD(6, d2, d3);
  };
  TileFeed feed(desc_of, *n_tiles);
  if constexpr (DB) {
    sweep_tiles_double_buffered<true>(feed, desc, metas, Abuf, load4, commit,
                                      [&](const TileMeta& m, const float4* __restrict__ A) { sweep(m, A, false); });
  } else {
    int di = 0;
    bool have = feed.pop(di);
    if (!have) return;
    tile_meta_store(metas[0], tile_meta_request(desc, di));
    for (int cur = 0; have; cur ^= 1) {
      TileMeta& m = metas[cur];
      sync_lds();
      have = feed.pop(di);
      int table_word = 0;
      if (have) table_word = tile_meta_request(desc, di);
      bool unsafe = EXACT && !exact_div_ok(c.h);
      if (!m.overflow) {
        StageRegs<3> sr;
        stage_issue<3>(m, load4, sr);
        commit(m, sr, Abuf[0]);
        if constexpr (EXACT) unsafe |= !stage_values_ok<3, 3>(m, sr);
      }
      if (have) tile_meta_store(metas[cur ^ 1], table_word);
      bool force_global = false;
      if constexpr (EXACT) {
        asm volatile("s_waitcnt lgkmcnt(0)" ::: "memory");
        force_global = __syncthreads_or(unsafe ? 1 : 0) != 0;
      }
      else sync_lds();
      sweep(m, Abuf[0], force_global);
    }
  }
}

constexpr int kPBlock = 256;
#ifndef DSL_PAIR_NINE
#define DSL_PAIR_NINE 1
#endif
constexpr bool kPairNine = DSL_PAIR_NINE != 0;
struct PairSlot {
  int srow, lx, g, own;
  int rowbase, j;
  bool two;
};
__device__ __forceinline__ PairSlot pair_slot(const TileMeta& m, int u) {
  const int ir = tile_row_of(m.pprefix, u);
  const int4 w = m.trow[ir];
  const int b1 = m.tprefix[ir], b2 = w.z & 0xffff, b3 = (int)((unsigned)w.z >> 16), b4 = w.w, b5 = m.tprefix[ir + 1];
  const int n1 = (b2 - b1 + 1) >> 1, n2 = (b3 - b2 + 1) >> 1, n3 = (b4 - b3 + 1) >> 1;
  int q = u - m.pprefix[ir];
  int lx = 1, begin = b1, end = b2;
  if (q >= n1) {
    q -= n1, lx = 2, begin = b2, end = b3;
    if (q >= n2) {
      q -= n2, lx = 3, begin = b3, end = b4;
      if (q >= n3) q -= n3, lx = 4, begin = b4, end = b5;
    }
  }
  const int t0 = begin + 2 * q;
  PairSlot r;
  r.srow = (ir / kTB + 1) * kTH + (ir % kTB + 1);
  r.lx = lx;
  r.g = w.x + t0;
  r.own = w.y + t0;
  r.rowbase = w.x;
  r.j = 2 * q;
  r.two = t0 + 1 < end;
  return r;
}

template <bool SHARE, bool WIDE = false>
__global__ __launch_bounds__(kPBlock, 4) void k_density_pair(DevConsts c, TileGrid tg, const int* __restrict__ desc_of,
                                                             const int* __restrict__ n_tiles, const int* __restrict__ desc,
                                                             const int* __restrict__ cell_start, Bnd bnd, CSoa3 p,
                                                             float* __restrict__ rho, float* __restrict__ pterm,
                                                             unsigned int* __restrict__ nmask, int mstride,
                                                             float wide_thr = 0.0f, SkinGate gate = SkinGate{nullptr}) {
  __shared__ TileMeta metas[2];
  __shared__ float4 A[kTCap];
  const int tid = threadIdx.x;
  if (gate.closed()) return;
  if (!WIDE && c.slab_axis < 0 && share_wanted(n_tiles) != SHARE) return;
  TileFeed feed(desc_of, *n_tiles);
  sweep_tiles_pair<kPBlock>(c, feed, desc, metas, A, p, [&](const TileMeta& m, bool ovf) {
    if (ovf) {
      if constexpr (!WIDE) {
        const int ntarg = m.tprefix[kTB * kTB];
        for (int t = tid; t < ntarg; t += kPBlock) {
          const int g = tile_target(m, t).g;
          const float a = bnd.is(g) ? 0.0f : density_global_fast(c, cell_start, p, g);
          store_density_fast(c, bnd, rho, pterm, g, a);
        }
      }
      return;
    }
    const int nslots = m.pprefix[kTB * kTB];
    for_each_target<SHARE, kPBlock, kPairNine>(nslots, tid, tid, [&](auto shared_c, int u, int sub, int k) {
      constexpr bool SHARED = decltype(shared_c)::value;
      const PairSlot ps = pair_slot(m, u);
      const int srow = ps.srow, lx = ps.lx, g0 = ps.g;
      const bool two = ps.two;
      float acc[2] = {0.0f, 0.0f}, accb[2] = {0.0f, 0.0f}, self_term[2] = {1.0f, 1.0f};
      const float4 me0 = A[ps.own];
      float4 me1 = A[ps.own + (two ? 1 : 0)];
      self_term[0] = (me0.x == me0.x && me0.y == me0.y && me0.z == me0.z) ? 1.0f : 0.0f;
      self_term[1] = (me1.x == me1.x && me1.y == me1.y && me1.z == me1.z) ? 1.0f : 0.0f;
      const float two_hh = 2.0f * c.inv_hh;
      const float sx0 = two_hh * me0.x, sy0 = two_hh * me0.y, sz0 = two_hh * me0.z, a00 = 1.0f + me0.w;
      const float sx1 = two_hh * me1.x, sy1 = two_hh * me1.y, sz1 = two_hh * me1.z;
      const float a01 = two ? 1.0f + me1.w : -1.0e30f;
      auto sweep_run = [&](int ri, int rr) {
        int j, je;
        tile_run(m, rr, lx, j, je);
        unsigned int mask0 = 0u, mask1 = 0u;
        auto test4 = [&](int jj) {
#pragma unroll
          for (int v = 0; v < 4; ++v) {
            const float4 cnd = A[jj + v];
            if constexpr (WIDE) {
              const float t0 = __builtin_fmaf(cnd.z, sz0, __builtin_fmaf(cnd.y, sy0, __builtin_fmaf(cnd.x, sx0, cnd.w + a00)));
              const float t1 = __builtin_fmaf(cnd.z, sz1, __builtin_fmaf(cnd.y, sy1, __builtin_fmaf(cnd.x, sx1, cnd.w + a01)));
              mask_push_lt(mask0, wide_thr, t0);
              mask_push_lt(mask1, wide_thr, t1);
              continue;
            }
            const float q0 = fma_clamp01(cnd.z, sz0, __builtin_fmaf(cnd.y, sy0, __builtin_fmaf(cnd.x, sx0, cnd.w + a00)));
            const float q1 = fma_clamp01(cnd.z, sz1, __builtin_fmaf(cnd.y, sy1, __builtin_fmaf(cnd.x, sx1, cnd.w + a01)));
            mask_push(mask0, q0);
            mask_push(mask1, q1);
            if (v & 1) {
              accb[0] = __builtin_fmaf(q0, q0, accb[0]);
              accb[1] = __builtin_fmaf(q1, q1, accb[1]);
            } else {
              acc[0] = __builtin_fmaf(q0, q0, acc[0]);
              acc[1] = __builtin_fmaf(q1, q1, acc[1]);
            }
          }
        };
        auto sweep_to = [&](int jend) {
          for (; j + 4 < jend; j += 8) {
            test4(j);
            test4(j + 4);
          }
          if (j < jend) {
            test4(j);
            j += 4;
          }
        };
        const int j32 = j + 32;
        sweep_to(min(je, j32));
        nmask[(size_t)ri * mstride + g0] = mask0;
        if (two) nmask[(size_t)ri * mstride + g0 + 1] = mask1;
        if (je > j32) {
          mask0 = mask1 = 0u;
          sweep_to(je);
          nmask[(size_t)(kMaskHigh + ri) * mstride + g0] = mask0;
          if (two) nmask[(size_t)(kMaskHigh + ri) * mstride + g0 + 1] = mask1;
        }
      };
      for_each_run<SHARED>(srow, sub, k, sweep_run);
      acc[0] += accb[0];
      acc[1] += accb[1];
      if constexpr (WIDE) return;
      if constexpr (SHARED) {
        if (k == 9) {
          acc[0] = nine_lane_sum(acc[0]);
          acc[1] = nine_lane_sum(acc[1]);
        } else {
          for (int o = 1; o < k; o <<= 1) {
            acc[0] += __shfl_xor(acc[0], o, kWave);
            acc[1] += __shfl_xor(acc[1], o, kWave);
          }
        }
        if (sub != 0) return;
      }
#pragma unroll
      for (int e = 0; e < 2; ++e) {
        if (e == 1 && !two) break;
        const int g = g0 + e;
        const float a = (acc[e] - self_term[e]) * (c.mass * c.A);
        store_density_fast(c, bnd, rho, pterm, g, a);
      }
    });
  });
}

constexpr int kOutIntegrate = 0, kOutAddForce = 1, kOutStore = 2, kOutPci = 3;

template <bool WANT_G, bool WANT_V, int OUT = kOutIntegrate, bool WANT_XS = false, bool SLAB = false, bool SHARE = true,
          bool EXACT = false, bool QUEUE = false>
__global__ __launch_bounds__(kTBlock, (WANT_G && WANT_V && !WANT_XS && !SLAB && !SHARE && !EXACT && OUT == kOutIntegrate) ? 1 : 4) void k_force_integrate_tiled(
    DevConsts c, TileGrid tg, const int* __restrict__ desc_of, const int* __restrict__ n_tiles,
    const int* __restrict__ ghost_desc_of, const int* __restrict__ n_ghost_tiles, const int* __restrict__ desc,
    const int* __restrict__ cell_start, CSoa3 pin, CSoa3 vin, const float* __restrict__ rho,
    const float* __restrict__ pterm, CSoa3 fin, int forces_uniform, Soa3 pout, Soa3 vout, DevStats* stats,
    const unsigned int* __restrict__ nmask, int mstride, const int* __restrict__ share_stats, Bnd bnd, Soa3 gout,
    int* __restrict__ walk_ctr = nullptr) {
  static_assert(!(EXACT && SHARE), "the exact sums are sequential: one lane per target");
  if (share_stats != nullptr && share_wanted(share_stats) != SHARE) return;
  __shared__ TileMeta metas[2];
  __shared__ float4 A[kTCap];
  __shared__ float4 B[kTCap];
  __shared__ int feed_slot[2];
  const int tid = threadIdx.x, lane = tid & (kWave - 1);
  unsigned int vbits = 0u, fbits = 0u;
  const int nphase = (SLAB && ghost_desc_of != nullptr) ? 2 : 1;
  for (int phase = 0; phase < nphase; ++phase) {
  const bool ghost_tile = phase == 1;
  static_assert(!(QUEUE && SLAB), "the tile queue walks list 0 of a single domain");
  typename TileSource<QUEUE>::type feed = TileSource<QUEUE>::make(ghost_tile ? ghost_desc_of : desc_of, ghost_tile ? *n_ghost_tiles : *n_tiles, walk_ctr, feed_slot);
  int di = 0;
  bool have = feed.pop(di);
  if (phase == 1) sync_lds();
  if (have) tile_meta_store(metas[0], tile_meta_request(desc, di));
  for (int cur = 0; have; cur ^= 1) {
    TileMeta& m = metas[cur];
    DSL_STAMP(t0);
    sync_lds();
    have = feed.pop(di);
    int table_word = 0;
    if (have) table_word = tile_meta_request(desc, di);
    DSL_STAMP(t1);
    DSL_STAMP_ADD(0, t0, t1);
    const bool ovf = m.overflow != 0;
    const bool nolds = ovf || ghost_tile;
    const int tperm = (tid & ~(kWave - 1)) + b128_group_slot(lane);
    unsigned int pre_word = 0u;
    if (!nolds && nmask != nullptr && tperm < m.tprefix[kTB * kTB]) {
      const int g0 = tile_target(m, tperm).g;
      pre_word = nmask[(size_t)(EXACT ? 0 : 4) * mstride + g0];
    }
    DSL_STAMP(t1b);
    DSL_STAMP_ADD(10, t1, t1b);
    bool unsafe = EXACT && !exact_div_ok(c.h);
    if (!nolds) {
      const bool values_ok = stage_rows<8, EXACT>(
          m,
          [&](int g, float4* o) {
            o[0] = load4u(pin.x + g);
            o[1] = load4u(pin.y + g);
            o[2] = load4u(pin.z + g);
            o[3] = (WANT_G || bnd.ids != nullptr) ? load4u(pterm + g) : make_float4(0.f, 0.f, 0.f, 0.f);
            if constexpr (WANT_V || WANT_XS) {
              o[4] = load4u(vin.x + g);
              o[5] = load4u(vin.y + g);
              o[6] = load4u(vin.z + g);
              o[7] = load4u(rho + g);
            } else {
              o[4] = o[5] = o[6] = o[7] = make_float4(0.f, 0.f, 0.f, 0.f);
            }
          },
          [&](int g, float* o) {
            o[0] = pin.x[g];
            o[1] = pin.y[g];
            o[2] = pin.z[g];
            o[3] = (WANT_G || bnd.ids != nullptr) ? pterm[g] : 0.f;
            if constexpr (WANT_V || WANT_XS) {
              o[4] = vin.x[g];
              o[5] = vin.y[g];
              o[6] = vin.z[g];
              o[7] = rho[g];
            }
          },
          [&](int slot, const float* o, bool real) {
            float4 a = make_float4(kFar, kFar, kFar, 0.f), b = make_float4(0.f, 0.f, 0.f, 0.f);
            if constexpr (EXACT) {
              if (real) {
// ... 832 lines not shown
```

dieselfluid_amd/csrc/sph_device.hpp:

```cpp
#pragma once

#include <hip/hip_runtime.h>
#include <stdint.h>

#include <type_traits>

namespace dsl {

constexpr int kWave = 64;

struct DevConsts {
  int n;
  float h, hh, inv_h, inv_hh, A, B, C, W0;
  float r2_thr;
  float mass, inv_mass, ref_density, mu, dt, delta;
  float eos_wg, eos_gamma, eos_d0_grad;
  float pressure_sign;
  int visc_running_mass;
  float reset[3], ext[3];
  int wcsph_pressure_force, wcsph_viscosity;
  float pci_max_error;
  float xsph_eps, st_kappa;
  int walls;
  float bmin[3], bmax[3], rest;
  float gmin[3];
  float inv_cell;
  float cell;
  int dims[3];
  int ncell;
  int slab_axis;
  float slab_lo, slab_hi;
  float chk_lo, chk_hi;
  int split_cl, split_ch;
  int split_part;
  int own_c0, own_c1;
  const int* n_ptr;
};

struct Soa3 {
  float *x, *y, *z;
};
struct CSoa3 {
  const float *x, *y, *z;
};

__device__ __forceinline__ int live_n(const DevConsts& c) { return c.n_ptr ? *c.n_ptr : c.n; }

struct Bnd {
  const int* ids;
  int n_fluid;
  __device__ __forceinline__ bool is(int slot) const { return ids != nullptr && ids[slot] >= n_fluid; }
};

struct DevStats {
  unsigned int max_vel_bits;
  unsigned int max_f_bits;
  unsigned int pci_cur_err_bits;
  unsigned int pci_last_err_bits;
  int pci_iters;
  int pci_done;
  int max_cell_count;
  int band_missed;
  int reserved0_;
  int pci_escaped;
};

struct SkinState {
  int rebuild;
  int ids_sel;
  float disp;
  unsigned int disp2_bits;
  int force;
  int n_steps, n_rebuilds;
  int list_overflow;
  float budget;
  float dt;
  unsigned int history;
  int give_up;
  int unlisted;
  int n_live;
  unsigned int fields_own, fields_padded;
  float tau;
  float predict;
  unsigned int vmax2_bits;
};
struct SkinGate {
  const SkinState* st;
  __device__ __forceinline__ bool closed() const { return st != nullptr && st->rebuild == 0; }
};

template <bool FAST>
__device__ __forceinline__ float dsl_sqrt(float x) {
  if constexpr (FAST) return __builtin_amdgcn_sqrtf(x);
  else return __builtin_sqrtf(x);
}
template <bool FAST>
__device__ __forceinline__ float dsl_div(float a, float b) {
  if constexpr (FAST) return a * __builtin_amdgcn_rcpf(b);
  else return a / b;
}

struct ExactDivisor {
  float d, r1;
};
__device__ __forceinline__ ExactDivisor exact_divisor(float d) {
  const float r0 = __builtin_amdgcn_rcpf(d);
  const float e0 = __builtin_fmaf(-d, r0, 1.0f);
  return ExactDivisor{d, __builtin_fmaf(e0, r0, r0)};
}
__device__ __forceinline__ ExactDivisor exact_divisor_uniform(float d) {
  const ExactDivisor D = exact_divisor(d);
  return ExactDivisor{__uint_as_float(__builtin_amdgcn_readfirstlane(__float_as_uint(D.d))),
                      __uint_as_float(__builtin_amdgcn_readfirstlane(__float_as_uint(D.r1)))};
}
__device__ __forceinline__ float exact_div(float n, const ExactDivisor& D) {
  const float q0 = n * D.r1;
  const float e1 = __builtin_fmaf(-D.d, q0, n);
  const float q1 = __builtin_fmaf(e1, D.r1, q0);
  const float e2 = __builtin_fmaf(-D.d, q1, n);
  const float q2 = __builtin_fmaf(e2, D.r1, q1);
  return __builtin_amdgcn_div_fixupf(q2, D.d, n);
}
__device__ __forceinline__ bool exact_div_ok(float v) {
  const float a = fabsf(v);
  return v == 0.0f || (a >= 0x1p-20f && a <= 0x1p20f);
}

template <bool FAST>
__device__ __forceinline__ float kern_F(const DevConsts& c, float dist) {
  if (dist >= c.h) return 0.0f;
  float xx = dist * dist;
  float q;
  if constexpr (FAST) q = __builtin_fmaf(-xx, c.inv_hh, 1.0f);
  else q = 1.0f - xx / c.hh;
  float aq = c.A * q;
  return aq * q;
}
template <bool FAST>
__device__ __forceinline__ float kern_O1D(const DevConsts& c, float dist) {
  if (dist >= c.h) return 0.0f;
  float q;
  if constexpr (FAST) q = __builtin_fmaf(-dist, c.inv_h, 1.0f);
  else q = 1.0f - dist / c.h;
  float bq = c.B * q;
  return bq * q;
}
template <bool FAST>
__device__ __forceinline__ float kern_O2D(const DevConsts& c, float dist) {
  if (dist > c.h) return 0.0f;
  float q;
  if constexpr (FAST) q = __builtin_fmaf(-dist, c.inv_h, 1.0f);
  else q = 1.0f - dist / c.h;
  return c.C * q;
}

template <bool FAST>
__device__ __forceinline__ float tait_eos(const DevConsts& c, float x, float d0) {
  if (x <= d0) x = d0;
  float ratio = dsl_div<FAST>(x, d0);
  float pw;
  if constexpr (FAST) {
    const float e = ratio - 1.0f;
    if (e <= 0.5f) {
      const float t = e * __builtin_amdgcn_rcpf(2.0f + e);
      const float t2 = t * t;
      float pl = 1.0f / 9.0f;
      pl = __builtin_fmaf(pl, t2, 1.0f / 7.0f);
      pl = __builtin_fmaf(pl, t2, 1.0f / 5.0f);
// ... 150 lines not shown
```

dieselfluid_amd/engine.py:

```python
from __future__ import annotations

import ctypes as C

import numpy as np

from ._lib import DslError, Params, Stats, load_library

BUF = {
    "positions": 0, "velocities": 1, "forces": 2, "densities": 3, "pressures": 4,
    "pci_positions": 5, "pci_velocities": 6,
}
_COMPS = {0: 3, 1: 3, 2: 3, 3: 1, 4: 1, 5: 3, 6: 3}
KERNEL_IDS = {
    "cell_rank": 0, "scan": 1, "scatter": 2, "density": 3, "force_integrate": 4, "pressure": 5, "viscous": 6,
    "gradient": 7, "external": 8, "update": 9, "pci_predict": 10, "pci_density": 11, "tile_list": 12,
    "neigh_lists": 13, "collide": 14,
}


def _fp(a):
    return a.ctypes.data_as(C.POINTER(C.c_float))


def reference_params(n3: int) -> Params:
# ... 381 lines not shown
    def pressure_all(self):
        self._ck(self._L.dsl_pressure_pass(self._h))

    def viscous_all(self):
        self._ck(self._L.dsl_viscous_pass(self._h))

    def external_all(self, f):
        a = np.ascontiguousarray(f, dtype=np.float32)
        self._ck(self._L.dsl_external_pass(self._h, _fp(a)))

    def gradient_pressure_force(self):
        self._ck(self._L.dsl_gradient_pressure_pass(self._h))

    def update(self):
        self._ck(self._L.dsl_update_pass(self._h))

    def force_pass(self):
        self._ck(self._L.dsl_force_pass(self._h))

    def set_collider_mesh(self, vertices=None, normals=None, radius: float = 0.0, restitution: float = 0.0):
        v = np.ascontiguousarray(vertices if vertices is not None else [], dtype=np.float32).reshape(-1)
        nrm = np.ascontiguousarray(normals if normals is not None else [], dtype=np.float32).reshape(-1)
        if v.size % 9 or nrm.size * 3 != v.size:
            raise DslError("set_collider_mesh: 9 vertex floats and 3 normal floats per triangle")
        self._ck(self._L.dsl_collider_set_mesh(self._h, _fp(v), _fp(nrm), v.size // 9, C.c_float(radius),
                                               C.c_float(restitution)))

    def collide(self):
        self._ck(self._L.dsl_collide_pass(self._h))

    def collider_query(self):
        n = self.n_fluid
        tri = np.empty(n, dtype=np.int32)
        nrm, coord, point = (np.empty((n, 3), dtype=np.float32) for _ in range(3))
        self._ck(self._L.dsl_collider_query(self._h, tri.ctypes.data_as(C.POINTER(C.c_int32)), _fp(nrm), _fp(coord),
                                            _fp(point)))
        return tri, nrm, coord, point

    def field_div(self, tensor: str = "velocities") -> np.ndarray:
        out = np.empty(self.n_fluid, dtype=np.float32)
        self._ck(self._L.dsl_field_divergence(self._h, BUF[tensor], _fp(out), out.size))
        return out

    def field_curl(self, tensor: str = "velocities") -> np.ndarray:
        out = np.empty(self.n_fluid * 3, dtype=np.float32)
        self._ck(self._L.dsl_field_curl(self._h, BUF[tensor], _fp(out), out.size))
        return out.reshape(-1, 3)

    def field_laplacian(self, scalar: str = "densities") -> np.ndarray:
        out = np.empty(self.n_fluid, dtype=np.float32)
        self._ck(self._L.dsl_field_laplacian(self._h, BUF[scalar], _fp(out), out.size))
        return out

    def field_interpolate(self, positions, scalar: str = "densities") -> np.ndarray:
        q = np.ascontiguousarray(positions, dtype=np.float32).reshape(-1, 3)
        out = np.empty(q.shape[0], dtype=np.float32)
        self._ck(self._L.dsl_field_interpolate(self._h, BUF[scalar], _fp(q), q.shape[0], _fp(out)))
        return out

    def wcsph_step(self, nsteps: int = 1):
        self._ck(self._L.dsl_wcsph_step(self._h, int(nsteps)))

    def pcisph_begin(self):
        self._ck(self._L.dsl_pcisph_begin(self._h))

    def pcisph_step(self, nsteps: int = 1):
        self._ck(self._L.dsl_pcisph_step(self._h, int(nsteps)))

    def sync(self):
        self._ck(self._L.dsl_sync(self._h))

    def stats(self) -> Stats:
        s = Stats()
        self._ck(self._L.dsl_get_stats(self._h, C.byref(s)))
        return s

    def timing_enable(self, on=True):
        self._ck(self._L.dsl_timing_enable(self._h, int(on)))

    def timing_reset(self):
        self._ck(self._L.dsl_timing_reset(self._h))

    OPTIONS = {"skin": 1, "skin_steps": 2, "skin_rebuilds": 3, "skin_list_overflow": 4, "skin_suspensions": 5, "device_bytes": 6, "skin_fields_own": 7, "skin_fields_padded": 8, "skin_predict": 9, "skin_tau_steps": 10,
               "density_pair": 16, "cell_keys": 17, "tile_box": 18, "persistent_blocks": 19, "pci_qtiled": 20,
               "pci_qpair": 21, "pci_qrows": 22, "pci_qincr": 23, "list_build": 24, "grid_oversub": 25, "tile_queue": 26,
               "collider_triangles": 32, "collide_hits": 33, "collide_cull": 34,
               "collide_index": 35, "collide_index_edge": 36, "collide_index_cells": 37, "collide_index_entries": 38,
               "collide_visits": 39, "collide_full_waves": 40, "collide_slab": 41}

    def set_option(self, name: str, value: float):
        self._ck(self._L.dsl_set_option(self._h, self.OPTIONS[name], float(value)))

    def get_option(self, name: str) -> float:
        v = C.c_double(0.0)
        self._ck(self._L.dsl_get_option(self._h, self.OPTIONS[name], C.byref(v)))
        return float(v.value)

    def timing(self, kernel: str):
        ms, cnt = C.c_double(0), C.c_int64(0)
        self._ck(self._L.dsl_timing_get(self._h, KERNEL_IDS[kernel], C.byref(ms), C.byref(cnt)))
        return ms.value, cnt.value
```

include/dslsph.h:

```cpp
#ifndef DSLSPH_H
#define DSLSPH_H

#include <stddef.h>
#include <stdint.h>

#ifdef __cplusplus
extern "C" {
#endif

#define DSL_ABI_VERSION 1

enum {
  DSL_OK = 0,
  DSL_ERR_INVALID = -1,
  DSL_ERR_DEVICE = -2,
  DSL_ERR_NOMEM = -3,
  DSL_ERR_UNSUPPORTED = -4,
  DSL_ERR_OVERFLOW = -5
};

enum {
  DSL_BUF_POSITIONS = 0,
  DSL_BUF_VELOCITIES = 1,
  DSL_BUF_FORCES = 2,
// ... 128 lines not shown
int dsl_collider_set_mesh(dsl_handle *h, const float *vertices , const float *normals ,
                          size_t n_triangles, float radius, float restitution);
int dsl_collide_pass(dsl_handle *h);
int dsl_collider_query(dsl_handle *h, int32_t *tri , float *normal ,
                       float *coord , float *point );

int dsl_get_stats(dsl_handle *h, dsl_stats *out);
int dsl_sync(dsl_handle *h);

int dsl_set_stream(dsl_handle *h, void *hip_stream);
int dsl_use_own_stream(dsl_handle *h);

int dsl_timing_enable(dsl_handle *h, int on);
int dsl_timing_reset(dsl_handle *h);
int dsl_timing_get(dsl_handle *h, int kernel_id, double *avg_ms, int64_t *launches);

int dsl_download_sorted(dsl_handle *h, int buffer, float *host, size_t count);
int dsl_download_ids(dsl_handle *h, int32_t *ids, size_t count);
int dsl_download_cell_start(dsl_handle *h, int32_t *cell_start, size_t count);

enum { DSL_SPLIT_BAND = 1, DSL_SPLIT_INNER = 2 };
size_t dsl_slab_message_floats(int cap_full, int cap_xonly);
int dsl_slab_record_floats(dsl_handle *h);
size_t dsl_slab_message_floats_for(dsl_handle *h, int cap_full, int cap_xonly);
int dsl_slab_config(dsl_handle *h, int axis, float lo, float hi);
int dsl_slab_split(dsl_handle *h, float width, float margin);
int dsl_slab_pack(dsl_handle *h, float width_full, float width, float *dev_lo, float *dev_hi, int cap_full,
                  int cap_xonly);
int dsl_slab_pack_band(dsl_handle *h, float width_full, float *dev_lo, float *dev_hi, int cap_full, int cap_xonly,
                       void *stream);
int dsl_force_pass_split(dsl_handle *h, int phase);
int dsl_slab_append(dsl_handle *h, const float *dev_message, int cap_full, int cap_xonly);
int dsl_slab_append2(dsl_handle *h, const float *dev_message_a, const float *dev_message_b, int cap_full,
                     int cap_xonly);
int dsl_slab_status(dsl_handle *h, int32_t status[4], int reset_high_water);
int dsl_slab_overflow(dsl_handle *h, int *high_water);
int dsl_get_count(dsl_handle *h, int *n_live, int *n_owned);
#define DSL_COMM_ID_BYTES 128
typedef struct dsl_comm dsl_comm;
int dsl_comm_unique_id(uint8_t id[DSL_COMM_ID_BYTES]);
int dsl_comm_create(int nranks, int rank, const uint8_t id[DSL_COMM_ID_BYTES], int device, dsl_comm **out);
int dsl_comm_create_all(int ndev, const int *devices, dsl_comm **out );
int dsl_comm_destroy(dsl_comm *c);
int dsl_comm_count(dsl_comm *c, int *nranks);
const char *dsl_comm_last_error(void);
typedef struct dsl_transport {
  void *ctx;
  int (*group_start)(void *ctx);
  int (*group_end)(void *ctx);
  int (*send)(void *ctx, const void *dev_buf, size_t bytes, int peer, void *stream);
  int (*recv)(void *ctx, void *dev_buf, size_t bytes, int peer, void *stream);
  int (*all_reduce_max_u32)(void *ctx, void *dev_buf , size_t count, void *stream);
} dsl_transport;
int dsl_comm_create_custom(int nranks, int rank, int device, const dsl_transport *transport, dsl_comm **out);
int dsl_create_multi(const dsl_params *params , int ndev, const int *devices, dsl_handle **handles ,
                     dsl_comm **comms );
int dsl_slab_attach(dsl_handle *h, dsl_comm *comm, int lo_rank, int hi_rank, float width_full, float width, int cap_full,
                    int cap_xonly, int overlap);
int dsl_slab_detach(dsl_handle *h);
int dsl_slab_image_shift(dsl_handle *h, float from_lo, float from_hi);
int dsl_slab_exchange(dsl_handle *h);
int dsl_slab_replan(dsl_handle *h);
int dsl_slab_wcsph_step(dsl_handle *h, int nsteps);
int dsl_slab_pcisph_step(dsl_handle *h, int nsteps);
int dsl_slab_layer_counts(dsl_handle *h, float origin, int n_layers, int32_t *dev_counts);
int dsl_slab_move_planes(dsl_handle *h, float lo, float hi);
int dsl_slab_get_planes(dsl_handle *h, float *lo, float *hi);
int dsl_slab_rebalance(dsl_handle *h, int every, float origin, int n_layers, const int32_t *planes ,
                       const int32_t *plane_min , const int32_t *plane_max , int min_layers);
int dsl_slab_rebalance_state(dsl_handle *h, int32_t *planes , int32_t *counts ,
                             int64_t *looks, int64_t *moves);

enum {
  DSL_OPT_SKIN = 1,
  DSL_OPT_SKIN_STEPS = 2,
  DSL_OPT_SKIN_REBUILDS = 3,
  DSL_OPT_SKIN_LIST_OVERFLOW = 4,
  DSL_OPT_SKIN_SUSPENSIONS = 5,
  DSL_OPT_DEVICE_BYTES = 6,
  DSL_OPT_SKIN_FIELDS_OWN = 7,
  DSL_OPT_SKIN_FIELDS_PADDED = 8,
  DSL_OPT_SKIN_PREDICT = 9,
  DSL_OPT_SKIN_TAU_STEPS = 10,
  DSL_OPT_DENSITY_PAIR = 16,
  DSL_OPT_CELL_KEYS = 17,
  DSL_OPT_TILE_BOX = 18,
  DSL_OPT_PERSISTENT_BLOCKS = 19,
  DSL_OPT_PCI_QTILED = 20,
  DSL_OPT_PCI_QPAIR = 21,
  DSL_OPT_PCI_QROWS = 22,
  DSL_OPT_LIST_BUILD = 24,
  DSL_OPT_GRID_OVERSUB = 25,
  DSL_OPT_TILE_QUEUE = 26,
  DSL_OPT_PCI_QINCR = 23,
  DSL_OPT_COLLIDER_TRIANGLES = 32,
  DSL_OPT_COLLIDE_HITS = 33,
  DSL_OPT_COLLIDE_CULL = 34,
  DSL_OPT_COLLIDE_INDEX = 35,
  DSL_OPT_COLLIDE_INDEX_EDGE = 36,
  DSL_OPT_COLLIDE_INDEX_CELLS = 37,
  DSL_OPT_COLLIDE_INDEX_ENTRIES = 38,
  DSL_OPT_COLLIDE_VISITS = 39,
  DSL_OPT_COLLIDE_FULL_WAVES = 40,
  DSL_OPT_COLLIDE_SLAB = 41
};
int dsl_set_option(dsl_handle *h, int option, double value);
int dsl_get_option(dsl_handle *h, int option, double *value);

int dsl_set_ids(dsl_handle *h, const int32_t *ids, size_t count);
int dsl_reset_forces(dsl_handle *h);

const char *dsl_last_error(dsl_handle *h);
const char *dsl_version(void);

#ifdef __cplusplus
}
#endif
#endif
```

Measured before the change: 8189 M particle-steps/s.

## Add per-particle Verlet skin budgets with packed float4 reference positions

Replaces the single uniform skin displacement budget with a per-particle budget stored in the w lane of a packed float4 reference-position array, double-buffered and selected via the skin state. Rebuild decisions now use a max displacement-to-budget ratio, and neighbour-list thresholds are widened per pair according to each particle's budget. The intent is to let slow particles hold tighter lists and fast particles looser ones, reducing list size or rebuild frequency. With the default floor of 1.0 the budgets stay uniform, so the main default effect is the changed reference layout (float4 AoS instead of three SoA arrays) plus extra per-pair threshold arithmetic.

```diff
diff --git a/bindings/go/dslsph/dslsph.go b/bindings/go/dslsph/dslsph.go
--- a/bindings/go/dslsph/dslsph.go
+++ b/bindings/go/dslsph/dslsph.go
@@ -429,6 +429,8 @@
 	OptSkinRebuilds    = int(C.DSL_OPT_SKIN_REBUILDS)
 	OptSkinSuspensions = int(C.DSL_OPT_SKIN_SUSPENSIONS)
 	OptSkinPredict     = int(C.DSL_OPT_SKIN_PREDICT)
+	OptSkinFloor       = int(C.DSL_OPT_SKIN_FLOOR)
+	OptSkinHeadroom    = int(C.DSL_OPT_SKIN_HEADROOM)
 	OptDeviceBytes     = int(C.DSL_OPT_DEVICE_BYTES)
 	OptGridOversub     = int(C.DSL_OPT_GRID_OVERSUB)
 	OptColliderTriangles = int(C.DSL_OPT_COLLIDER_TRIANGLES)
diff --git a/dieselfluid_amd/csrc/dslsph.hip b/dieselfluid_amd/csrc/dslsph.hip
--- a/dieselfluid_amd/csrc/dslsph.hip
+++ b/dieselfluid_amd/csrc/dslsph.hip
@@ -644,7 +644,7 @@
   (void)hipFree(h->walk_ctr);
   (void)hipFree(h->lists);
   for (int k = 0; k < 6; ++k) (void)hipFree(h->pvz[k]);
-  for (int k = 0; k < 3; ++k) (void)hipFree(h->pvr[k]);
+  for (int k = 0; k < 2; ++k) (void)hipFree(h->pvr[k]);
   (void)hipFree(h->stage);
   (void)hipFree(h->dstats);
   (void)hipFree(h->dcounter);
@@ -1324,7 +1324,7 @@
   if (!h->lists && (rc = dev_alloc(h, &h->lists, (size_t)kLMaxChunks * h->cap))) return rc;
   for (int k = 0; k < 6; ++k)
     if (!h->pvz[k] && (rc = dev_alloc(h, &h->pvz[k], (size_t)h->cap))) return rc;
-  for (int k = 0; k < 3; ++k)
+  for (int k = 0; k < 2; ++k)
     if (!h->pvr[k] && (rc = dev_alloc(h, &h->pvr[k], (size_t)h->cap))) return rc;
   return DSL_OK;
 }
@@ -1347,6 +1347,12 @@
   init.dt = h->c.dt;
   init.n_live = h->n;
   init.predict = h->skin_predict;
+  init.budget_full = 0.5f * h->skin * h->c.h;
+  init.ref[0] = h->pvr[0];
+  init.ref[1] = h->pvr[1];
+  init.floor = h->skin_floor;
+  init.headroom = h->skin_headroom;
+  init.uniform = 1;
   init.vmax2_bits = 0x7f800000u;
   HIP_TRY(h, hipMemcpyAsync(h->skin_state, &init, sizeof(init), hipMemcpyHostToDevice, h->stream));
   HIP_TRY(h, hipStreamSynchronize(h->stream));
@@ -1363,8 +1369,8 @@
   const int X = h->cur_pv, Y = X ^ 1;
   const CSoa3 pX = cpos(h), vX = cvel(h);
   const CSoa3 pZ{h->pvz[0], h->pvz[1], h->pvz[2]}, vZ{h->pvz[3], h->pvz[4], h->pvz[5]};
-  const CSoa3 pR{h->pvr[0], h->pvr[1], h->pvr[2]};
-  const Soa3 pRw{h->pvr[0], h->pvr[1], h->pvr[2]};
+  const CSoa3 no3{nullptr, nullptr, nullptr};
+  const Soa3 no3w{nullptr, nullptr, nullptr};
   const bool ordered = sort_ordered(h);
   hipLaunchKernelGGL(k_skin_decide, dim3(1), dim3(1), 0, h->stream, st);
   HIP_TRY(h, hipGetLastError());
@@ -1388,26 +1394,25 @@
                   ordered ? h->cell_keys : nullptr, h->dcounter + 3};
   rc = timed(h, DSL_K_SCATTER, [&] {
     hipLaunchKernelGGL(HIP_KERNEL_NAME(k_scatter<true, 6>), dim3(std::min(grid_for((n + kScatterUnroll - 1) / kScatterUnroll), 4096)), dim3(kBlock), 0, h->stream, c, a, so, pX, h->rank, h->cell_start, gate,
-                       vX, pRw);
+                       vX, no3w);
     if (ordered)
       hipLaunchKernelGGL(k_scatter_ordered<true>, dim3(h->cell_keys ? std::min(grid_for(n), 1024) : grid_for(n)), dim3(kBlock), 0,
-                         h->stream, c, a, so, pX, h->rank, h->cell_start, gate, vX, pRw);
+                         h->stream, c, a, so, pX, h->rank, h->cell_start, gate, vX, no3w);
   });
   if (rc) return rc;
   rc = timed(h, DSL_K_TILE_LIST, [&] { launch_tile_tables(h, nullptr, gate); });
   if (rc) return rc;
-  const double reach = 1.0 + (double)h->skin;
-  const float wide_thr = (float)(1.0 - reach * reach * 1.0004 - 1.0e-4);
+  const float wide_thr = skin_wide_thr(h->skin);
   rc = timed(h, DSL_K_NEIGH_LISTS, [&] {
     hipLaunchKernelGGL((k_density_pair<true, true>), dim3(persistent_grid(h, 8, true)), dim3(kPBlock), 0, h->stream, c, h->tg,
-                       h->tile_desc_of, h->n_tiles, h->tile_desc, h->cell_start, bnd_of(h), pR, h->rho, h->pterm, h->nmask,
+                       h->tile_desc_of, h->n_tiles, h->tile_desc, h->cell_start, bnd_of(h), no3, h->rho, h->pterm, h->nmask,
                        h->cap, wide_thr, gate);
     if (h->list_build_lockstep)
       hipLaunchKernelGGL(k_list_build, dim3(persistent_grid(h, 2, true)), dim3(kLBlock), 0, h->stream, c, h->tg, h->tile_desc_of,
-                         h->n_tiles, h->tile_desc, h->nmask, h->cap, h->lists, h->cap, st, gate, pR, wide_thr);
+                         h->n_tiles, h->tile_desc, h->nmask, h->cap, h->lists, h->cap, st, gate, no3, wide_thr);
     else
       hipLaunchKernelGGL(k_list_build_v1, dim3(persistent_grid(h, 2, true)), dim3(kLBlock), 0, h->stream, c, h->tg, h->tile_desc_of,
-                         h->n_tiles, h->tile_desc, h->nmask, h->cap, h->lists, h->cap, st, gate, pR, wide_thr);
+                         h->n_tiles, h->tile_desc, h->nmask, h->cap, h->lists, h->cap, st, gate, no3, wide_thr);
   });
   if (rc) return rc;
   rc = timed(h, DSL_K_DENSITY, [&] {
@@ -1423,7 +1428,7 @@
     with_flag(G, [&](auto fg) { with_flag(V, [&](auto fv) { with_flag(wql != nullptr, [&](auto fq) {
       constexpr bool GG = decltype(fg)::value, VV = decltype(fv)::value || !GG;
       hipLaunchKernelGGL((k_force_list<GG, VV, decltype(fq)::value>), g, b, 0, h->stream, c, h->tg, h->tile_desc_of, h->n_tiles,
-                         h->tile_desc, h->cell_start, st, pX, vX, pZ, vZ, pR, h->rho, h->pterm, h->lists, h->cap, po, vo, h->dstats,
+                         h->tile_desc, h->cell_start, st, pX, vX, pZ, vZ, no3, h->rho, h->pterm, h->lists, h->cap, po, vo, h->dstats,
                          wql);
     }); }); });
   });
@@ -1498,6 +1503,14 @@
     case DSL_OPT_SKIN_PREDICT:
       if (!(value >= 0.0 && value <= 0.95)) return fail(h, DSL_ERR_INVALID, "dsl_set_option: DSL_OPT_SKIN_PREDICT is a fraction of the displacement budget in [0, 0.95]");
       h->skin_predict = (float)value;
+      return DSL_OK;
+    case DSL_OPT_SKIN_FLOOR:
+      if (!(value > 0.0 && value <= 1.0)) return fail(h, DSL_ERR_INVALID, "dsl_set_option: DSL_OPT_SKIN_FLOOR is a fraction of the displacement budget in (0, 1]");
+      h->skin_floor = (float)value;
+      return DSL_OK;
+    case DSL_OPT_SKIN_HEADROOM:
+      if (!(value >= 1.05 && value <= 4.0)) return fail(h, DSL_ERR_INVALID, "dsl_set_option: DSL_OPT_SKIN_HEADROOM is a factor in [1.05, 4]");
+      h->skin_headroom = (float)value;
       return DSL_OK;
     case DSL_OPT_DENSITY_PAIR: h->density_pair = value != 0.0; return DSL_OK;
     case DSL_OPT_CELL_KEYS:
@@ -1583,6 +1596,8 @@
     case DSL_OPT_SKIN_FIELDS_OWN: *value = (double)s.fields_own; return DSL_OK;
     case DSL_OPT_SKIN_FIELDS_PADDED: *value = (double)s.fields_padded; return DSL_OK;
     case DSL_OPT_SKIN_PREDICT: *value = h->skin_predict; return DSL_OK;
+    case DSL_OPT_SKIN_FLOOR: *value = h->skin_floor; return DSL_OK;
+    case DSL_OPT_SKIN_HEADROOM: *value = h->skin_headroom; return DSL_OK;
     case DSL_OPT_SKIN_TAU_STEPS: *value = s.dt > 0.0f ? (double)s.tau / (double)s.dt : 0.0; return DSL_OK;
     case DSL_OPT_DENSITY_PAIR: *value = h->density_pair ? 1.0 : 0.0; return DSL_OK;
     case DSL_OPT_CELL_KEYS: *value = h->cell_keys != nullptr ? 1.0 : 0.0; return DSL_OK;
diff --git a/dieselfluid_amd/csrc/engine.hpp b/dieselfluid_amd/csrc/engine.hpp
--- a/dieselfluid_amd/csrc/engine.hpp
+++ b/dieselfluid_amd/csrc/engine.hpp
@@ -14,6 +14,8 @@
 
 namespace dsl {
 constexpr float kSkinPredict = 0.8f;
+constexpr float kSkinFloor = 1.0f;
+constexpr float kSkinHeadroom = 1.25f;
 }
 
 struct dsl_handle {
@@ -96,8 +98,10 @@
   dsl::SkinState* skin_state = nullptr;
   uint4* lists = nullptr;
   float* pvz[6] = {};
-  float* pvr[3] = {};
+  float4* pvr[2] = {};
   float skin_predict = dsl::kSkinPredict;
+  float skin_floor = dsl::kSkinFloor;
+  float skin_headroom = dsl::kSkinHeadroom;
   bool list_build_lockstep = true;
   int grid_oversub = 8;
   int tile_queue = 1;
diff --git a/dieselfluid_amd/csrc/kernels_grid.hpp b/dieselfluid_amd/csrc/kernels_grid.hpp
--- a/dieselfluid_amd/csrc/kernels_grid.hpp
+++ b/dieselfluid_amd/csrc/kernels_grid.hpp
@@ -229,21 +229,37 @@
 
 struct SortPos {
   float x, y, z;
+  float b;
 };
 template <bool REF>
 __device__ __forceinline__ SortPos sort_pos(const CSoa3& pos, const CSoa3& vel, float tau, int i) {
-  if constexpr (REF) return SortPos{skin_ref(pos.x[i], vel.x[i], tau), skin_ref(pos.y[i], vel.y[i], tau), skin_ref(pos.z[i], vel.z[i], tau)};
-  return SortPos{pos.x[i], pos.y[i], pos.z[i]};
+  if constexpr (REF) return SortPos{skin_ref(pos.x[i], vel.x[i], tau), skin_ref(pos.y[i], vel.y[i], tau), skin_ref(pos.z[i], vel.z[i], tau), 0.0f};
+  return SortPos{pos.x[i], pos.y[i], pos.z[i], 0.0f};
+}
+struct SkinBudgetRule {
+  float B, floor, headroom;
+  bool predict;
+};
+__device__ __forceinline__ SkinBudgetRule skin_budget_rule(const SkinState* st) {
+  return SkinBudgetRule{st->budget_full, st->floor, st->headroom, st->uniform == 0 && st->floor < 1.0f};
+}
+__device__ __forceinline__ float skin_budget_at(const SkinBudgetRule& r, const SkinRef& old, int i, float x, float y, float z,
+                                                const SortPos& sp) {
+  if (!r.predict) return r.B;
+  const float4 o = old.r[i];
+  const float ex = x - o.x, ey = y - o.y, ez = z - o.z;
+  const float ax = sp.x - x, ay = sp.y - y, az = sp.z - z;
+  const float d = __builtin_sqrtf(__builtin_fmaf(ez, ez, __builtin_fmaf(ey, ey, ex * ex)));
+  const float a = __builtin_sqrtf(__builtin_fmaf(az, az, __builtin_fmaf(ay, ay, ax * ax)));
+  return skin_budget_of(r.B, r.floor, r.headroom, d, a);
 }
 template <bool REF>
 __device__ __forceinline__ void scatter_move(const ScatterArrays& a, const ScatterOrder& o, int i, int d, int id,
-                                             int* __restrict__ ids_dst, const Soa3& ref, const SortPos& sp) {
+                                             int* __restrict__ ids_dst, const SkinRef& ref, const SortPos& sp) {
   ids_dst[d] = id;
   for (int f = 0; f < a.nf; ++f) a.dst[f][d] = a.src[f][i];
   if constexpr (REF) {
-    ref.x[d] = sp.x;
-    ref.y[d] = sp.y;
-    ref.z[d] = sp.z;
+    ref.r[d] = make_float4(sp.x, sp.y, sp.z, sp.b);
   }
   if (o.dest) o.dest[i] = d;
 }
@@ -270,16 +286,14 @@
 }
 template <bool REF, int NFMAX>
 __device__ __forceinline__ void scatter_store(const ScatterArrays& a, const ScatterOrder& o, int i, int d, int id,
-                                              int* __restrict__ ids_dst, const Soa3& ref, const SortPos& sp,
+                                              int* __restrict__ ids_dst, const SkinRef& ref, const SortPos& sp,
                                               const ScatterPayload<NFMAX>& p) {
   ids_dst[d] = id;
 #pragma unroll
   for (int f = 0; f < NFMAX; ++f)
     if (NFMAX == 6 || f < a.nf) a.dst[f][d] = p.v[f];
   if constexpr (REF) {
-    ref.x[d] = sp.x;
-    ref.y[d] = sp.y;
-    ref.z[d] = sp.z;
+    ref.r[d] = make_float4(sp.x, sp.y, sp.z, sp.b);
   }
   if (o.dest) o.dest[i] = d;
 }
@@ -293,13 +307,15 @@
                                                     const int* __restrict__ rank,
                                                     const int* __restrict__ cell_start, SkinGate gate = SkinGate{nullptr},
                                                     CSoa3 vel = CSoa3{nullptr, nullptr, nullptr},
-                                                    Soa3 ref = Soa3{nullptr, nullptr, nullptr}) {
+                                                    Soa3 = Soa3{nullptr, nullptr, nullptr}) {
   constexpr int U = kScatterUnroll;
   if (gate.closed()) return;
   const ScatterIds ids = skin_ids(a, gate);
   const int* ids_src = ids.src;
   int* ids_dst = ids.dst;
   const float tau = REF ? gate.st->tau : 0.0f;
+  const SkinRef ref = REF ? skin_ref_set(gate.st) : SkinRef{nullptr}, ref_old = REF ? skin_ref_set(gate.st, false) : SkinRef{nullptr};
+  const SkinBudgetRule rule = REF ? skin_budget_rule(gate.st) : SkinBudgetRule{0.0f, 1.0f, 1.0f, false};
   const int n = live_n(c);
   const bool pos_in_payload = a.nf >= (REF ? 6 : 3) && pos.x == a.src[0] && pos.y == a.src[1] && pos.z == a.src[2] &&
                               (!REF || (vel.x == a.src[3] && vel.y == a.src[4] && vel.z == a.src[5]));
@@ -317,10 +333,12 @@
     id[u] = ids_src[i];
     r[u] = rank[i];
     if (pos_in_payload) {
-      if constexpr (REF) sp[u] = SortPos{skin_ref(pay[u].v[0], pay[u].v[3], tau), skin_ref(pay[u].v[1], pay[u].v[4], tau), skin_ref(pay[u].v[2], pay[u].v[5], tau)};
-      else sp[u] = SortPos{pay[u].v[0], pay[u].v[1], pay[u].v[2]};
+      if constexpr (REF) sp[u] = SortPos{skin_ref(pay[u].v[0], pay[u].v[3], tau), skin_ref(pay[u].v[1], pay[u].v[4], tau), skin_ref(pay[u].v[2], pay[u].v[5], tau), 0.0f};
+      else sp[u] = SortPos{pay[u].v[0], pay[u].v[1], pay[u].v[2], 0.0f};
+      if constexpr (REF) sp[u].b = skin_budget_at(rule, ref_old, i, pay[u].v[0], pay[u].v[1], pay[u].v[2], sp[u]);
     } else {
       sp[u] = sort_pos<REF>(pos, vel, tau, i);
+      if constexpr (REF) sp[u].b = skin_budget_at(rule, ref_old, i, pos.x[i], pos.y[i], pos.z[i], sp[u]);
     }
   }
 #pragma unroll
@@ -371,15 +389,17 @@
                                                             const int* __restrict__ cell_start,
                                                             SkinGate gate = SkinGate{nullptr},
                                                             CSoa3 vel = CSoa3{nullptr, nullptr, nullptr},
-                                                            Soa3 ref = Soa3{nullptr, nullptr, nullptr}) {
+                                                            Soa3 = Soa3{nullptr, nullptr, nullptr}) {
   if (gate.closed()) return;
   const ScatterIds ids = skin_ids(a, gate);
   const float tau = REF ? gate.st->tau : 0.0f;
+  const SkinRef ref = REF ? skin_ref_set(gate.st) : SkinRef{nullptr}, ref_old = REF ? skin_ref_set(gate.st, false) : SkinRef{nullptr};
+  const SkinBudgetRule rule = REF ? skin_budget_rule(gate.st) : SkinBudgetRule{0.0f, 1.0f, 1.0f, false};
   if (o.cell_keys != nullptr) {
     if (*o.overfull == 0) return;
     const int n = live_n(c);
     for (int i = blockIdx.x * kBlock + threadIdx.x; i < n; i += gridDim.x * kBlock) {
-      const SortPos sp = sort_pos<REF>(pos, vel, tau, i);
+      SortPos sp = sort_pos<REF>(pos, vel, tau, i);
       const int cell = sort_cell(c, sp.x, sp.y, sp.z);
       if (cell == c.ncell) continue;
       const int s = cell_start[cell], e = cell_start[cell + 1];
@@ -390,13 +410,15 @@
         const int key = o.keys[k];
         below += (key < id || (key == id && k < mine)) ? 1 : 0;
       }
+      if constexpr (REF) sp.b = skin_budget_at(rule, ref_old, i, pos.x[i], pos.y[i], pos.z[i], sp);
       scatter_move<REF>(a, o, i, s + below, id, ids.dst, ref, sp);
     }
     return;
   }
   const int i = blockIdx.x * kBlock + threadIdx.x;
   if (i >= live_n(c) || !o.later[i]) return;
-  const SortPos sp = sort_pos<REF>(pos, vel, tau, i);
+  SortPos sp = sort_pos<REF>(pos, vel, tau, i);
+  if constexpr (REF) sp.b = skin_budget_at(rule, ref_old, i, pos.x[i], pos.y[i], pos.z[i], sp);
   const int cell = sort_cell(c, sp.x, sp.y, sp.z);
   const int id = ids.src[i];
   const int s = cell_start[cell], e = cell_start[cell + 1], mine = s + rank[i];
diff --git a/dieselfluid_amd/csrc/kernels_skin.hpp b/dieselfluid_amd/csrc/kernels_skin.hpp
--- a/dieselfluid_amd/csrc/kernels_skin.hpp
+++ b/dieselfluid_amd/csrc/kernels_skin.hpp
@@ -15,12 +15,14 @@
 
 __global__ void k_skin_decide(SkinState* st) {
   const float d = __builtin_sqrtf(__uint_as_float(st->disp2_bits)) * (1.0f + 1.0e-6f);
-  const bool rb = st->force != 0 || !(d <= st->budget);
+  const float ratio = __builtin_sqrtf(__uint_as_float(st->ratio2_bits)) * (1.0f + 1.0e-6f);
+  const bool rb = st->force != 0 || !(ratio <= 1.0f - 1.0e-3f);
   st->rebuild = rb ? 1 : 0;
   if (st->unlisted * 64 > st->n_live) st->give_up = 1;
   if (rb) {
     st->ids_sel ^= 1;
     st->n_rebuilds += 1;
+    st->uniform = st->force != 0 ? 1 : 0;
     st->unlisted = 0;
     st->fields_own = st->fields_padded = 0u;
     const float vmax = __builtin_sqrtf(__uint_as_float(st->vmax2_bits)) * (1.0f + 1.0e-6f);
@@ -31,6 +33,7 @@
   st->disp = d;
   st->force = 0;
   st->disp2_bits = 0u;
+  st->ratio2_bits = 0u;
   st->vmax2_bits = 0u;
   st->n_steps += 1;
   st->history = (st->history << 1) | (rb ? 1u : 0u);
@@ -43,8 +46,10 @@
                                                         const int* __restrict__ n_tiles, const int* __restrict__ desc,
                                                         const unsigned int* __restrict__ nmask, int mstride,
                                                         uint4* __restrict__ lists, int lstride, SkinState* st,
-                                                        SkinGate gate, CSoa3 p, float wide_thr) {
+                                                        SkinGate gate, CSoa3, float wide_thr) {
   if (gate.closed()) return;
+  const SkinRef p = skin_ref_set(st);
+  const SkinSplit split{wide_thr, c.h, st->budget_full, c.inv_hh};
   __shared__ TileMeta metas[2];
   constexpr int kLStaged = 8;
   __shared__ uint4 held[kLStaged][kLBlock];
@@ -104,11 +109,13 @@
           if (len > 64) {
             const int rr = tt.srow + (ri / 3 - 1) * kTH + (ri % 3 - 1);
             const int g0 = m.row_gs[rr] - m.row_lds[rr];
-            const float xi = p.x[g], yi = p.y[g], zi = p.z[g];
+            const float4 me = p.r[g];
+            const float xi = me.x, yi = me.y, zi = me.z, thr = skin_thr(split, me.w);
             for (int r = j; r < je; ++r) {
-              const float dx = xi - p.x[g0 + r], dy = yi - p.y[g0 + r], dz = zi - p.z[g0 + r];
-              const float tq = __builtin_fmaf(-dist2<true>(dx, dy, dz), c.inv_hh, 1.0f);
-              if (tq > wide_thr) emit(r);
+              const float4 o = p.r[g0 + r];
+              const float dx = xi - o.x, dy = yi - o.y, dz = zi - o.z;
+              const float tq = __builtin_fmaf(-dist2<true>(dx, dy, dz), c.inv_hh, 1.0f) - skin_ej(split, o.w);
+              if (tq > thr) emit(r);
             }
             continue;
           }
@@ -168,7 +175,7 @@
                                                         const int* __restrict__ n_tiles, const int* __restrict__ desc,
                                                         const unsigned int* __restrict__ nmask, int mstride,
                                                         uint4* __restrict__ lists, int lstride, SkinState* st,
-                                                        SkinGate gate, CSoa3 p, float wide_thr) {
+                                                        SkinGate gate, CSoa3, float wide_thr) {
   if (gate.closed()) return;
   __shared__ TileMeta metas[2];
   __shared__ unsigned int qword[kLQueue][kLBlock];
@@ -241,14 +248,18 @@
           int j, je;
           tile_run(m, rr, tt.lx, j, je);
           const int g0 = m.row_gs[rr] - m.row_lds[rr];
-          const float xi = p.x[g], yi = p.y[g], zi = p.z[g];
+          const SkinRef p = skin_ref_set(st);
+          const SkinSplit split{wide_thr, c.h, st->budget_full, c.inv_hh};
+          const float4 me = p.r[g];
+          const float xi = me.x, yi = me.y, zi = me.z, thr = skin_thr(split, me.w);
           for (int r0 = j; r0 < je; r0 += 32) {
             unsigned int w = 0u;
             const int top = r0 + 31;
             for (int r = r0; r < min(r0 + 32, je); ++r) {
-              const float dx = xi - p.x[g0 + r], dy = yi - p.y[g0 + r], dz = zi - p.z[g0 + r];
-              const float tq = __builtin_fmaf(-dist2<true>(dx, dy, dz), c.inv_hh, 1.0f);
-              if (tq > wide_thr && r != tt.own) w |= 1u << (top - r);
+              const float4 o = p.r[g0 + r];
+              const float dx = xi - o.x, dy = yi - o.y, dz = zi - o.z;
+              const float tq = __builtin_fmaf(-dist2<true>(dx, dy, dz), c.inv_hh, 1.0f) - skin_ej(split, o.w);
+              if (tq > thr && r != tt.own) w |= 1u << (top - r);
             }
             enqueue(w, top);
           }
@@ -521,7 +532,7 @@
 __global__ __launch_bounds__(kLBlock, 4) void k_force_list(DevConsts c, TileGrid tg, const int* __restrict__ desc_of,
                                                            const int* __restrict__ n_tiles, const int* __restrict__ desc,
                                                            const int* __restrict__ cell_start, SkinState* st, CSoa3 pX,
-                                                           CSoa3 vX, CSoa3 pZ, CSoa3 vZ, CSoa3 pR, const float* __restrict__ rho,
+                                                           CSoa3 vX, CSoa3 pZ, CSoa3 vZ, CSoa3, const float* __restrict__ rho,
                                                            const float* __restrict__ pterm,
                                                            const uint4* __restrict__ lists, int lstride, Soa3 pout,
                                                            Soa3 vout, DevStats* stats, int* __restrict__ walk_ctr) {
@@ -532,7 +543,8 @@
   const int tid = threadIdx.x;
   const bool rb = st->rebuild != 0;
   const CSoa3 pin = rb ? pZ : pX, vin = rb ? vZ : vX;
-  unsigned int vbits = 0u, fbits = 0u, dbits = 0u;
+  const SkinRef pR = skin_ref_set(st);
+  unsigned int vbits = 0u, fbits = 0u, dbits = 0u, qbits = 0u;
   typename TileSource<QUEUE>::type feed = TileSource<QUEUE>::make(desc_of, *n_tiles, walk_ctr, feed_slot);
   int di = 0;
   bool have = feed.pop(di);
@@ -742,9 +754,12 @@
       fz += c.ext[2];
       integrate_core(c, fx, fy, fz, px, py, pz, vx, vy, vz, vbits, fbits);
       {
-        const float ex = px - pR.x[g], ey = py - pR.y[g], ez = pz - pR.z[g];
-        const unsigned int db = nonneg_bits(__builtin_fmaf(ez, ez, __builtin_fmaf(ey, ey, ex * ex)));
+        const float4 rf = pR.r[g];
+        const float ex = px - rf.x, ey = py - rf.y, ez = pz - rf.z, bi = rf.w;
+        const float d2 = __builtin_fmaf(ez, ez, __builtin_fmaf(ey, ey, ex * ex));
+        const unsigned int db = nonneg_bits(d2), qb = nonneg_bits(d2 * __builtin_amdgcn_rcpf(bi * bi));
         dbits = db > dbits ? db : dbits;
+        qbits = qb > qbits ? qb : qbits;
       }
       pout.x[g] = px;
       pout.y[g] = py;
@@ -758,6 +773,7 @@
   wave_atomic_max(&stats->max_vel_bits, vbits);
   wave_atomic_max(&stats->max_f_bits, fbits);
   wave_atomic_max(&st->disp2_bits, dbits);
+  wave_atomic_max(&st->ratio2_bits, qbits);
   wave_atomic_max(&st->vmax2_bits, vbits);
 }
 
diff --git a/dieselfluid_amd/csrc/kernels_tiled.hpp b/dieselfluid_amd/csrc/kernels_tiled.hpp
--- a/dieselfluid_amd/csrc/kernels_tiled.hpp
+++ b/dieselfluid_amd/csrc/kernels_tiled.hpp
@@ -772,12 +772,10 @@
   }
 }
 
-template <int BLOCK, class Body>
-__device__ __forceinline__ void sweep_tiles_pair(const DevConsts& c, TileFeed& feed, const int* desc, TileMeta* metas,
-                                                 float4* A, const CSoa3& p, Body&& body) {
+template <int BLOCK, int NF, class Load4, class Load1, class MakeStore, class Body>
+__device__ __forceinline__ void sweep_tiles_pair_from(TileFeed& feed, const int* desc, TileMeta* metas, const Load4& load4,
+                                                      const Load1& load1, MakeStore&& make_store, Body&& body) {
   const int tid = threadIdx.x;
-  const LoadPos4 load4{p};
-  const LoadPos1 load1{p};
   auto meta_request = [&](int desc_index, int (&w)[2]) {
 #pragma unroll
     for (int k = 0; k < 2; ++k) {
@@ -808,18 +806,54 @@
     if (have) meta_request(di, tw);
     const bool ovf = m.overflow != 0;
     if (!ovf) {
-      const StoreTileRecord store(A, m, c.inv_hh);
-      StageRegs<3> sr0, sr1;
-      stage_issue<3>(m, load4, sr0, tid);
-      stage_issue<3>(m, load4, sr1, tid + BLOCK);
-      stage_commit<3>(m, sr0, load1, store, tid);
-      stage_commit<3>(m, sr1, load1, store, tid + BLOCK);
+      const auto store = make_store(m);
+      StageRegs<NF> sr0, sr1;
+      stage_issue<NF>(m, load4, sr0, tid);
+      stage_issue<NF>(m, load4, sr1, tid + BLOCK);
+      stage_commit<NF>(m, sr0, load1, store, tid);
+      stage_commit<NF>(m, sr1, load1, store, tid + BLOCK);
     }
     if (have) meta_store(metas[cur ^ 1], tw);
     sync_lds();
     body(m, ovf);
   }
 }
+template <int BLOCK, class Body>
+__device__ __forceinline__ void sweep_tiles_pair(const DevConsts& c, TileFeed& feed, const int* desc, TileMeta* metas,
+                                                 float4* A, const CSoa3& p, Body&& body) {
+  sweep_tiles_pair_from<BLOCK, 3>(feed, desc, metas, LoadPos4{p}, LoadPos1{p},
+                                  [&](const TileMeta& m) { return StoreTileRecord(A, m, c.inv_hh); }, body);
+}
+
+struct LoadRef4 {
+  SkinRef r;
+  __device__ __forceinline__ void operator()(int g, float4* o) const {
+    const float4 t0 = r.r[g], t1 = r.r[g + 1], t2 = r.r[g + 2], t3 = r.r[g + 3];
+    o[0] = make_float4(t0.x, t1.x, t2.x, t3.x);
+    o[1] = make_float4(t0.y, t1.y, t2.y, t3.y);
+    o[2] = make_float4(t0.z, t1.z, t2.z, t3.z);
+    o[3] = make_float4(t0.w, t1.w, t2.w, t3.w);
+  }
+};
+struct LoadRef1 {
+  SkinRef r;
+  __device__ __forceinline__ void operator()(int g, float* o) const {
+    const float4 t = r.r[g];
+    o[0] = t.x;
+    o[1] = t.y;
+    o[2] = t.z;
+    o[3] = t.w;
+  }
+};
+struct StoreRefRecord {
+  StoreTileRecord plain;
+  SkinSplit split;
+  __device__ __forceinline__ void operator()(int slot, const float* o, bool real) const {
+    float4 v = tile_record(o, real, plain.ox, plain.oy, plain.oz, plain.inv_hh);
+    if (real) v.w -= skin_ej(split, o[3]);
+    plain.img[slot] = v;
+  }
+};
 struct MaskQueue {
   unsigned int mm, n1, n2;
   int top, tp1, tp2;
@@ -1156,9 +1190,15 @@
   __shared__ float4 A[kTCap];
   const int tid = threadIdx.x;
   if (gate.closed()) return;
+  SkinRef ref{nullptr};
+  SkinSplit split{0.0f, 0.0f, 0.0f, 0.0f};
+  if constexpr (WIDE) {
+    ref = skin_ref_set(gate.st);
+    split = SkinSplit{wide_thr, c.h, gate.st->budget_full, c.inv_hh};
+  }
   if (!WIDE && c.slab_axis < 0 && share_wanted(n_tiles) != SHARE) return;
   TileFeed feed(desc_of, *n_tiles);
-  sweep_tiles_pair<kPBlock>(c, feed, desc, metas, A, p, [&](const TileMeta& m, bool ovf) {
+  auto sweep = [&](const TileMeta& m, bool ovf) {
     if (ovf) {
       if constexpr (!WIDE) {
         const int ntarg = m.tprefix[kTB * kTB];
@@ -1185,6 +1225,12 @@
       const float sx0 = two_hh * me0.x, sy0 = two_hh * me0.y, sz0 = two_hh * me0.z, a00 = 1.0f + me0.w;
       const float sx1 = two_hh * me1.x, sy1 = two_hh * me1.y, sz1 = two_hh * me1.z;
       const float a01 = two ? 1.0f + me1.w : -1.0e30f;
+      float thr0 = 0.0f, thr1 = 0.0f;
+      if constexpr (WIDE) {
+        const float b0 = ref.r[g0].w, b1 = ref.r[g0 + (two ? 1 : 0)].w;
+        thr0 = skin_thr(split, b0) - skin_ej(split, b0);
+        thr1 = skin_thr(split, b1) - skin_ej(split, b1);
+      }
       auto sweep_run = [&](int ri, int rr) {
         int j, je;
         tile_run(m, rr, lx, j, je);
@@ -1196,8 +1242,8 @@
             if constexpr (WIDE) {
               const float t0 = __builtin_fmaf(cnd.z, sz0, __builtin_fmaf(cnd.y, sy0, __builtin_fmaf(cnd.x, sx0, cnd.w + a00)));
               const float t1 = __builtin_fmaf(cnd.z, sz1, __builtin_fmaf(cnd.y, sy1, __builtin_fmaf(cnd.x, sx1, cnd.w + a01)));
-              mask_push_lt(mask0, wide_thr, t0);
-              mask_push_lt(mask1, wide_thr, t1);
+              mask_push_lt(mask0, thr0, t0);
+              mask_push_lt(mask1, thr1, t1);
               continue;
             }
             const float q0 = fma_clamp01(cnd.z, sz0, __builtin_fmaf(cnd.y, sy0, __builtin_fmaf(cnd.x, sx0, cnd.w + a00)));
@@ -1258,7 +1304,11 @@
         store_density_fast(c, bnd, rho, pterm, g, a);
       }
     });
-  });
+  };
+  if constexpr (WIDE)
+    sweep_tiles_pair_from<kPBlock, 4>(feed, desc, metas, LoadRef4{ref}, LoadRef1{ref},
+                                      [&](const TileMeta& m) { return StoreRefRecord{StoreTileRecord(A, m, c.inv_hh), split}; }, sweep);
+  else sweep_tiles_pair<kPBlock>(c, feed, desc, metas, A, p, sweep);
 }
 
 constexpr int kOutIntegrate = 0, kOutAddForce = 1, kOutStore = 2, kOutPci = 3;
diff --git a/dieselfluid_amd/csrc/skin_budget.hpp b/dieselfluid_amd/csrc/skin_budget.hpp
--- /dev/null
+++ b/dieselfluid_amd/csrc/skin_budget.hpp
@@ -0,0 +1,28 @@
+#pragma once
+
+#if defined(__HIPCC__) || defined(__CUDACC__)
+#define DSL_SKIN_HD __host__ __device__ inline
+#else
+#define DSL_SKIN_HD inline
+#endif
+
+namespace dsl {
+
+inline float skin_wide_thr(float s) {
+  const double reach = 1.0 + (double)s;
+  return (float)(1.0 - reach * reach * 1.0004 - 1.0e-4);
+}
+
+struct SkinSplit {
+  float wide_thr, h, B, inv_hh;
+};
+DSL_SKIN_HD float skin_ej(const SkinSplit& s, float bj) { return (s.B - bj) * (2.0f * (s.h + s.B) + s.B + bj) * s.inv_hh; }
+DSL_SKIN_HD float skin_thr(const SkinSplit& s, float bi) { return s.wide_thr + (s.B - bi) * (2.0f * s.h + s.B + bi) * s.inv_hh; }
+
+DSL_SKIN_HD float skin_budget_of(float B, float floor_, float headroom, float d, float a) {
+  const float want = headroom * (d > a ? d : a);
+  const float lo = floor_ * B;
+  return !(want > lo) ? lo : (want > B ? B : want);
+}
+
+}
diff --git a/dieselfluid_amd/csrc/sph_device.hpp b/dieselfluid_amd/csrc/sph_device.hpp
--- a/dieselfluid_amd/csrc/sph_device.hpp
+++ b/dieselfluid_amd/csrc/sph_device.hpp
@@ -4,6 +4,8 @@
 #include <stdint.h>
 
 #include <type_traits>
+
+#include "skin_budget.hpp"
 
 namespace dsl {
 
@@ -83,7 +85,19 @@
   float tau;
   float predict;
   unsigned int vmax2_bits;
-};
+  float budget_full;
+  float floor, headroom;
+  int uniform;
+  unsigned int ratio2_bits;
+  float4* ref[2];
+};
+struct SkinRef {
+  float4* r;
+};
+__device__ __forceinline__ SkinRef skin_ref_set(const SkinState* st, bool current = true) {
+  const bool second = (st->ids_sel != 0) == current;
+  return SkinRef{second ? st->ref[1] : st->ref[0]};
+}
 struct SkinGate {
   const SkinState* st;
   __device__ __forceinline__ bool closed() const { return st != nullptr && st->rebuild == 0; }
diff --git a/dieselfluid_amd/engine.py b/dieselfluid_amd/engine.py
--- a/dieselfluid_amd/engine.py
+++ b/dieselfluid_amd/engine.py
@@ -487,6 +487,7 @@
         self._ck(self._L.dsl_timing_reset(self._h))
 
     OPTIONS = {"skin": 1, "skin_steps": 2, "skin_rebuilds": 3, "skin_list_overflow": 4, "skin_suspensions": 5, "device_bytes": 6, "skin_fields_own": 7, "skin_fields_padded": 8, "skin_predict": 9, "skin_tau_steps": 10,
+               "skin_floor": 11, "skin_headroom": 12,
                "density_pair": 16, "cell_keys": 17, "tile_box": 18, "persistent_blocks": 19, "pci_qtiled": 20,
                "pci_qpair": 21, "pci_qrows": 22, "pci_qincr": 23, "list_build": 24, "grid_oversub": 25, "tile_queue": 26,
                "collider_triangles": 32, "collide_hits": 33, "collide_cull": 34,
diff --git a/include/dslsph.h b/include/dslsph.h
--- a/include/dslsph.h
+++ b/include/dslsph.h
@@ -234,6 +234,8 @@
   DSL_OPT_SKIN_FIELDS_PADDED = 8,
   DSL_OPT_SKIN_PREDICT = 9,
   DSL_OPT_SKIN_TAU_STEPS = 10,
+  DSL_OPT_SKIN_FLOOR = 11,
+  DSL_OPT_SKIN_HEADROOM = 12,
   DSL_OPT_DENSITY_PAIR = 16,
   DSL_OPT_CELL_KEYS = 17,
   DSL_OPT_TILE_BOX = 18,
```

Result: no change. 8197 M particle-steps/s, median of 4 (+0.1%).
